# leakless21/VietVoice-TTS

Measured on AMD Instinct MI355X. Metric: audio-seconds/sec (24 kHz) at batch 32, 256-token utterances; RTF, higher is better.
Workload: dtype bf16

## Files before the change

### include/vvtts.h

```cpp
#ifndef VVTTS_H
#define VVTTS_H
#include <stddef.h>
#include <stdint.h>

#ifdef __cplusplus
extern "C" {
#endif

#if defined(__GNUC__)
#define VV_API __attribute__((visibility("default")))
#else
#define VV_API
#endif

#define VV_DTYPE_F32 0
#define VV_DTYPE_BF16 1
#define VV_MAX_UP 8
#define VV_MAX_RES 4

#define VV_ACT_NONE_ 0
#define VV_ACT_GELU_TANH_ 1
#define VV_ACT_GELU_ERF_ 2
#define VV_ACT_SILU_ 3
#define VV_ACT_MISH_ 4
// ... 103 lines not shown
    const float* t_host;
} vv_apg_args;
VV_API int vv_transformer_steps_apg(vv_ctx* ctx, const vv_steps_args* args, const uint8_t* guide_host, int ld_guide, const vv_apg_args* apg,
                                    void* stream);
VV_API int vv_transformer_apg_ws_bytes(vv_ctx* ctx, int B, int N, const int32_t* seq_len_host, uint64_t* bytes);

VV_API int vv_decode_ws_bytes(vv_ctx* ctx, int B, int t_gen_max, uint64_t* bytes);
VV_API int vv_decode_into(vv_ctx* ctx, int B, int N, const float* x, const int32_t* ref_signal_len, const int32_t* seq_len,
                   int t_gen_max, int16_t* pcm, int ld_pcm, int32_t* pcm_len, float* wave_f32, void* ws, uint64_t ws_bytes,
                   void* stream);
VV_API uint64_t vv_ws_generation(const vv_ctx* ctx);

VV_API int vv_set_rope_theta(vv_ctx* ctx, float theta);

VV_API int vv_set_option(vv_ctx* ctx, const char* name, int value);

#define VV_PROF_GEMM 0
#define VV_PROF_ATTN 1
#define VV_PROF_NORM 2
#define VV_PROF_POSCONV 3
#define VV_PROF_ELEMWISE 4
#define VV_PROF_VOC_CONV 5
#define VV_PROF_VOC_POST 6
#define VV_PROF_MEL 7
#define VV_PROF_TEXT 8
#define VV_PROF_VOC_PRE 9
#define VV_PROF_VOC_UP0 10
#define VV_PROF_VOC_MRF0 14
#define VV_PROF_NCLASS 18
VV_API int vv_prof_enable(vv_ctx* ctx, int on);
VV_API int vv_prof_collect(vv_ctx* ctx, int64_t* launches, double* ms, double* flops, double* bytes);

typedef struct vv_gemm_args {
    int32_t dtype, out_dtype, mode, act;
    const void* A; int32_t lda;
    const void* W; int32_t ldw;
    void* C; int32_t ldc;
    int32_t M, N, K;
    const float *bias, *gate, *cos_q, *sin_q, *cos_k, *sin_k;
    int32_t n_store, seq_n, rope_dim;
    const float *rope_cs_q, *rope_cs_k;
    int32_t tile;
    const int32_t* rope_pos;
    int32_t rope_by_row;
    int32_t tail_parts, tail_row0;
    void* C_tail;
    float rope_theta;
    int32_t rope_skip_q;
    int32_t chip_share;
} vv_gemm_args;
VV_API int vv_gemm(vv_ctx* ctx, const vv_gemm_args* args, void* stream);
VV_API int vv_gemm_tail_plan(vv_ctx* ctx, int32_t M, int32_t N, int32_t K, int32_t* row0, int32_t* parts);

typedef struct vv_attn_args {
    int32_t dtype;
    const void* qkv; int32_t ld_qkv;
    void* out; int32_t ld_out;
    int32_t n_seq, seq_n, heads, dim;
    const int32_t* kv_len;
    const int32_t* row_start;
    int32_t total_rows;
    float q_scale;
    const float* rope_cs_q;
} vv_attn_args;
VV_API int vv_attention(vv_ctx* ctx, const vv_attn_args* args, void* stream);

typedef struct vv_ln_args {
    int32_t out_dtype;
    const float* x; int32_t ldx;
    void* y; int32_t ldy;
    int32_t R, D;
    const float *w, *b;
    int32_t add_one;
    float eps;
    const void* delta;
    int32_t delta_dtype, ld_delta;
    const void* delta2;
    int32_t keep_x;
    int32_t tail_row0;
    int32_t delta_tail_parts, delta2_tail_parts;
    const void *delta_tail, *delta2_tail;
} vv_ln_args;
VV_API int vv_layernorm(vv_ctx* ctx, const vv_ln_args* args, void* stream);

typedef struct vv_posconv_args {
    int32_t dtype, out_dtype;
    const void* in; int32_t ld_in;
    const void* W;
    const float* bias;
    void* out; int32_t ld_out;
    const void* resid; int32_t ld_resid;
    int32_t n_seq, seq_n, groups, KW, B;
    const int32_t* seq_len;
    const int32_t* row_start;
} vv_posconv_args;
VV_API int vv_posconv(vv_ctx* ctx, const vv_posconv_args* args, void* stream);

typedef struct vv_conv_args {
    const float* in;
    const float* W;
    const float* bias;
    float* out;
    const float* resid;
    int32_t B, Cin, Cout, T_in, T_out, KW, dil, transposed, up, rows_total, rows_pad, accumulate;
    float pre_slope, out_scale;
    const int32_t* len_in;
    const void* W_x3;
    int32_t wg_rows;
} vv_conv_args;
VV_API int vv_conv1d(vv_ctx* ctx, const vv_conv_args* args, void* stream);
VV_API uint64_t vv_conv_split_bytes(int32_t Cin_pad, int32_t KW, int32_t rows_pad);
VV_API int vv_conv_split_weights(vv_ctx* ctx, const float* W, int32_t Cin_pad, int32_t KW, int32_t rows_pad, void* out, void* stream);

typedef struct vv_mrf_args {
    const float* y;
    const float *W1, *b1;
    const float *W2, *b2;
    float* out;
    int32_t B, C, T, KW, dil, rows_pad, accumulate;
    float slope, out_scale;
    const int32_t* len_in;
} vv_mrf_args;
VV_API int vv_mrf_resblock(vv_ctx* ctx, const vv_mrf_args* args, void* stream);

VV_API int vv_vocos_im2col(vv_ctx* ctx, const float* x, int B, int N, const int32_t* ref_signal_len, const int32_t* seq_len, int T_max,
                           float* out, int ld_out, void* stream);
VV_API int vv_istft_head(vv_ctx* ctx, int B, int T_max, const float* head, int ld_head, const int32_t* n_frames, int16_t* pcm, int ld_pcm,
                         int32_t* pcm_len, float* wave_f32, void* stream);
VV_API int vv_text_embed(vv_ctx* ctx, const int32_t* ids, int ld_ids, const int32_t* text_len, const float* emb, const float* pos,
                         int vocab_rows, float* out, int B, int N, int Dt, void* stream);
VV_API int vv_dwconv(vv_ctx* ctx, const float* in, float* out, const float* w, const float* bias, const int32_t* seq_len, int B, int n_seq,
                     int N, int C, int KW, void* stream);
VV_API int vv_grn(vv_ctx* ctx, int dtype, void* x, float* sumsq, const float* gamma, const float* beta, const int32_t* seq_len, int B,
                  int n_seq, int N, int C, void* stream);
VV_API int vv_conv_post(vv_ctx* ctx, const float* in, const float* w, float bias, int16_t* pcm, int ld_pcm, float* wave_f32,
                 int B, int C, int T, int KW, float pre_slope, const int32_t* len_in, void* stream);
VV_API int vv_mel(vv_ctx* ctx, const int16_t* audio, int ld_audio, const int32_t* audio_len, float* mel, int B, int F_max,
           void* stream);
VV_API int vv_groupnorm(vv_ctx* ctx, const float* x, float* y, const float* gamma, const float* beta, int B, int C, int T, int G,
                 float eps, int act, void* stream);
VV_API int vv_rope_compact(vv_ctx* ctx, const float* cos_t, const float* sin_t, float* out, int n, void* stream);
VV_API int vv_rope_rows(vv_ctx* ctx, const float* compact, const int32_t* pos, float* out, int rows, void* stream);
typedef struct vv_ode_stage_args {
    float* x; const float* pred; int32_t ldp, Rc, n_mel, n_prev;
    const float* k_prev[3]; float coef[4];
    float* k_out; float* x_out;
    float g; const float* g_item; int32_t seq_n; const int32_t* row_src;
} vv_ode_stage_args;
VV_API int vv_ode_stage(vv_ctx* ctx, const vv_ode_stage_args* args, void* stream);
VV_API int vv_ode_stage_guided(vv_ctx* ctx, const vv_ode_stage_args* args, const int32_t* u_row, void* stream);
typedef struct vv_apg_coef_args {
    const float* pred; int32_t ldp, Rc, n_mel;
    const int32_t* u_row;
    const float* x_e; const int32_t* row_src;
    int32_t B, n_tiles;
    const int32_t* row_start; const int32_t* len;
    float t_e, g;
    const float* g_item; const float* eta; const float* norm_rms;
    double* partials; float* coef;
} vv_apg_coef_args;
VV_API int vv_apg_coef(vv_ctx* ctx, const vv_apg_coef_args* args, void* stream);
typedef struct vv_apg_stage_args { const float* coef; const float* x_e; int32_t x_e_packed; float t_e; } vv_apg_stage_args;
VV_API int vv_ode_stage_apg(vv_ctx* ctx, const vv_ode_stage_args* args, const int32_t* u_row, const vv_apg_stage_args* apg, void* stream);
VV_API int vv_cfg_euler(vv_ctx* ctx, float* x, const float* pred, int ldp, int BN, int n_mel, float cfg, float dt, void* stream);

VV_API int vv_ingest_pcm(vv_ctx* ctx, const void* pcm, const int64_t* desc, int n_clips, int64_t max_out, float* out, void* stream);
// ... 56 lines not shown
```

### vietvoice-tts_amd/csrc/vv_api.hip

```cpp
#include <hip/hip_runtime.h>
#include <algorithm>
#include <cmath>
#include <cstdarg>
#include <cstdio>
#include <cstring>
#include <map>
#include <string>
#include <utility>
#include <vector>
#include "vv_kernels.h"

#define VV_VERSION_STR "vvtts-hip 0.9 (gfx950)"

namespace {
std::string g_create_error;

struct Bound { const void* p; uint64_t bytes; };

struct ProfRec { hipEvent_t a, b; int cls, sub; };

inline size_t align_up(size_t v, size_t a) { return (v + a - 1) / a * a; }
inline int pad_to(int v, int a) { return (v + a - 1) / a * a; }
}

struct vv_ctx {
    int device = 0;
    vv_model_cfg cfg{};
    int dt = VV_DTYPE_BF16;
    std::string err;
    std::map<std::string, Bound> w;
    bool finalized = false;
    bool ever_finalized = false;
    bool vocos = false;
    vv_vocos_cfg vcfg{};
    float post_bias = 0.f;
    int n_steps = 0;
    std::vector<float> dt_host;
    float* modtab = nullptr;
    float* fintab = nullptr;
    int ode_s = 1;
    double ode_a[16] = {}, ode_b[4] = {1.0, 0, 0, 0};
    int ode_kslot[4] = {-1, -1, -1, -1};
    int ode_nk = 0;
    char* ws = nullptr;
    size_t ws_cap = 0;
    uint64_t ws_generation = 0;
    int* d_mult = nullptr;
    int rope_rows = 0;
    int split_k_tail = 0;
    int chip_share = 1;
    int ring_tiles_max = 256;
    int ring_tiles = 1;
    int pp_min_tiles = -1;
    int lanes = 0;
    hipStream_t side_stream[1] = {};
    hipEvent_t ev_fork = nullptr, ev_join[1] = {};
    float rope_theta = 0.f;
    int rope_q_attn = 1;
    int voc_x3 = -1;
    int voc_x3_rows = 0;
    char* x3_buf = nullptr;
    std::map<std::string, const void*> x3_w;
    int fuse_mrf = 2;
    bool prof = false;
    std::vector<ProfRec> recs;
    std::vector<hipEvent_t> pool;
    int64_t p_launch[VV_PROF_NCLASS]{};
    double p_flops[VV_PROF_NCLASS]{}, p_bytes[VV_PROF_NCLASS]{}, p_ms[VV_PROF_NCLASS]{};

    int fail(int code, const char* fmt, ...) {
        char buf[1024];
        va_list ap;
        va_start(ap, fmt);
        vsnprintf(buf, sizeof buf, fmt, ap);
        va_end(ap);
        err = buf;
        return code;
    }
    const void* W(const std::string& n) const {
        auto it = w.find(n);
        return it == w.end() ? nullptr : it->second.p;
    }
    const float* Wf(const std::string& n) const { return (const float*)W(n); }
    int esz() const { return dt == VV_DTYPE_BF16 ? 2 : 4; }
    int bk() const { return dt == VV_DTYPE_BF16 ? 64 : 32; }
};

namespace {

#define HIPCHK(ctx, call)                                                                   \
    do {                                                                                    \
        hipError_t e__ = (call);                                                            \
        if (e__ != hipSuccess) return (ctx)->fail(-5, "%s: %s", #call, hipGetErrorString(e__)); \
    } while (0)

#define KCHK(ctx, call)                                              \
    do {                                                             \
        const char* m__ = "";                                        \
        int r__ = (call);                                            \
        if (r__ != 0) return (ctx)->fail(r__, "%s", m__);            \
    } while (0)

struct Prof {
    vv_ctx* c; int idx = -1; hipStream_t st;
    Prof(vv_ctx* c_, int cls, double flops, double bytes, hipStream_t st_, int sub = -1) : c(c_), st(st_) {
        if (!c->prof) return;
        ProfRec r; r.cls = cls; r.sub = sub;
        if (sub >= 0) { c->p_launch[sub]++; c->p_flops[sub] += flops; c->p_bytes[sub] += bytes; }
        auto get = [&]() { hipEvent_t e; if (!c->pool.empty()) { e = c->pool.back(); c->pool.pop_back(); } else hipEventCreate(&e); return e; };
        r.a = get(); r.b = get();
        hipEventRecord(r.a, st);
        c->recs.push_back(r); idx = (int)c->recs.size() - 1;
        c->p_launch[cls]++; c->p_flops[cls] += flops; c->p_bytes[cls] += bytes;
    }
    ~Prof() { if (idx >= 0) hipEventRecord(c->recs[idx].b, st); }
};

struct Arena {
    char* base = nullptr; size_t cap = 0, off = 0;
    template <typename T> T* take(size_t n) { off = align_up(off, 256); T* p = base ? (T*)(base + off) : nullptr; off += n * sizeof(T); return p; }
};
template <typename F> size_t plan_bytes(F&& plan) { Arena dry; plan(dry); return dry.off; }
int ensure_ws(vv_ctx* c, size_t bytes, Arena* a) {
    if (bytes > c->ws_cap) {
        if (c->ws) { hipDeviceSynchronize(); hipFree(c->ws); c->ws = nullptr; c->ws_cap = 0; }
        const size_t want = align_up(bytes + bytes / 16, 1 << 20);
        hipError_t e = hipMalloc((void**)&c->ws, want);
        if (e != hipSuccess) return c->fail(-12, "workspace hipMalloc(%zu MiB): %s", want >> 20, hipGetErrorString(e));
        c->ws_cap = want; ++c->ws_generation;
    }
    *a = Arena{c->ws, c->ws_cap, 0};
    return 0;
}
int use_ws(vv_ctx* c, void* block, size_t have, size_t need, Arena* a) {
    if ((uintptr_t)block % 256) return c->fail(-22, "workspace block must be 256-byte aligned");
    if (have < need) return c->fail(-22, "workspace block too small: %zu < %zu bytes", have, need);
    *a = Arena{(char*)block, have, 0};
    return 0;
}
template <typename F> int plan_ws(vv_ctx* c, void* block, size_t have, F&& plan) {
    const size_t need = plan_bytes(plan);
    Arena a;
    if (int r = block ? use_ws(c, block, have, need, &a) : ensure_ws(c, need, &a)) return r;
    plan(a);
    if (a.off > a.cap) return c->fail(-14, "workspace plan took %zu bytes of a %zu-byte block", a.off, a.cap);
    return 0;
}

struct Gemm : vv_gemm_args { const char* wname; };
Gemm gemm_args(const vv_ctx* c, int dtype, int out_dtype, int mode, int act, const void* A, int lda, const char* wname, int ldw,
               const char* bname, void* C, int ldc, int M, int N, int K) {
    Gemm g{};
    g.dtype = dtype; g.out_dtype = out_dtype; g.mode = mode; g.act = act;
    g.A = A; g.lda = lda; g.W = c->W(wname); g.ldw = ldw; g.C = C; g.ldc = ldc; g.M = M; g.N = N; g.K = K;
    g.bias = bname ? c->Wf(bname) : nullptr; g.wname = wname;
    if (bname && !g.bias) g.W = nullptr;
    return g;
}
int launch_gemm(vv_ctx* c, Gemm g, int cls, hipStream_t st, double alg_flops = -1) {
    if (!g.W) return c->fail(-2, "weight '%s' is not bound", g.wname);
    const int M = g.M, N = g.N, K = g.K, bf16 = g.dtype == VV_DTYPE_BF16;
    if (!g.chip_share) g.chip_share = c->chip_share;
    if (g.tile == 0 && c->pp_min_tiles >= 0 && bf16 && N % 256 == 0)
        g.tile = (M >= 4096 && (long long)((M + 255) / 256) * (N / 256) >= c->pp_min_tiles) ? 256 : 128;
    if (c->ring_tiles && g.tile == 0 && bf16 && N <= 1024 && N % 64 == 0 && (long long)((M + 63) / 64) * (N / 128) <= c->ring_tiles_max)
        g.tile = 6464;
    const int esz = bf16 ? 2 : 4, osz = g.out_dtype == VV_DTYPE_BF16 ? 2 : 4;
    const double fl = alg_flops >= 0 ? alg_flops : 2.0 * M * (double)N * K;
    Prof p(c, cls, fl, (double)M * K * esz + (double)N * K * esz + (double)M * N * osz * (g.mode == VV_EPI_GATE_RES ? 2 : 1), st);
    const char* m = "";
    if (int r = vvk_gemm(&g, st, &m)) return c->fail(r, "%s (weight %s, M=%d N=%d K=%d)", m, g.wname, M, N, K);
    return 0;
}

std::string blk(int i, const char* s) { return "blocks." + std::to_string(i) + s; }

}

extern "C" {

const char* vv_version(void) { return VV_VERSION_STR; }

const char* vv_last_error(const vv_ctx* ctx) { return ctx ? ctx->err.c_str() : g_create_error.c_str(); }

int vv_create(vv_ctx** out, int device, const vv_model_cfg* cfg, int acoustic_dtype) {
    if (!out || !cfg) { g_create_error = "vv_create: null argument"; return -22; }
    *out = nullptr;
    int n = 0;
    hipError_t e = hipGetDeviceCount(&n);
    if (e != hipSuccess || n <= 0) { g_create_error = "vv_create: no HIP device visible (the HIP path has no CPU fallback)"; return -19; }
    if (device < 0 || device >= n) { g_create_error = "vv_create: device index out of range"; return -22; }
    if (acoustic_dtype != VV_DTYPE_F32 && acoustic_dtype != VV_DTYPE_BF16) { g_create_error = "vv_create: dtype must be f32 or bf16"; return -22; }
    if (cfg->head_dim != 64 || cfg->heads * 64 != cfg->dim) { g_create_error = "vv_create: head_dim must be 64"; return -22; }
    if (cfg->dim % 128 || cfg->text_dim % 128 || cfg->dim / cfg->pos_conv_groups != 64 || cfg->n_mel % 4 || cfg->dim > 1024 ||
        cfg->text_dim > 1024) {
        g_create_error = "vv_create: dim/text_dim must be multiples of 128 (<=1024), 64 channels per pos-conv group"; return -22;
    }
    if (cfg->voc_n_up < 1 || cfg->voc_n_up > VV_MAX_UP || cfg->voc_n_res > VV_MAX_RES || cfg->voc_n_dil > VV_MAX_RES) {
        g_create_error = "vv_create: vocoder topology out of range"; return -22;
    }
    e = hipSetDevice(device);
    if (e != hipSuccess) { g_create_error = hipGetErrorString(e); return -5; }
    vv_ctx* c = new vv_ctx();
    c->device = device; c->cfg = *cfg; c->dt = acoustic_dtype;
    *out = c;
    return 0;
}

void vv_destroy(vv_ctx* c) {
    if (!c) return;
    hipSetDevice(c->device);
    hipDeviceSynchronize();
    if (c->ws) hipFree(c->ws);
    if (c->modtab) hipFree(c->modtab);
    if (c->fintab) hipFree(c->fintab);
    if (c->d_mult) hipFree(c->d_mult);
    if (c->x3_buf) hipFree(c->x3_buf);
    for (auto q : c->side_stream) if (q) hipStreamDestroy(q);
    if (c->ev_fork) hipEventDestroy(c->ev_fork);
    for (auto e : c->ev_join) if (e) hipEventDestroy(e);
    for (auto& r : c->recs) { hipEventDestroy(r.a); hipEventDestroy(r.b); }
    for (auto e : c->pool) hipEventDestroy(e);
    delete c;
}

int vv_bind_weight(vv_ctx* c, const char* name, const void* p, uint64_t bytes) {
    if (!c || !name || !p) return c ? c->fail(-22, "vv_bind_weight: null argument") : -22;
    if ((uintptr_t)p % 16) return c->fail(-22, "vv_bind_weight(%s): pointer must be 16-byte aligned", name);
    c->w[name] = Bound{p, bytes};
    c->finalized = false;
    return 0;
}

int vv_finalize_weights(vv_ctx* c) {
    if (!c) return -22;
    const vv_model_cfg& g = c->cfg;
    const int D = g.dim, Dt = g.text_dim, FF = g.dim * g.ff_mult, es = c->esz();
    const int KP = pad_to(2 * g.n_mel + Dt, 64), MP = pad_to(g.n_mel, 128);
    std::string missing;
    auto need = [&](const std::string& n, uint64_t bytes) {
        auto it = c->w.find(n);
        if (it == c->w.end()) { missing += n + " "; return; }
        if (it->second.bytes < bytes) missing += n + "(short:" + std::to_string(it->second.bytes) + "<" + std::to_string(bytes) + ") ";
    };
    need("const.window", 4ull * g.n_fft); need("const.tw_cos", 4ull * g.n_fft); need("const.tw_sin", 4ull * g.n_fft);
    need("const.mel_fb", 4ull * (g.n_fft / 2 + 1) * g.n_mel);
    need("const.text_pos", 4ull * g.max_pos * Dt);
    need("text.embed.weight", 4ull * g.vocab_rows * Dt);
    for (int i = 0; i < g.text_layers; ++i) {
        const std::string p = "text.blocks." + std::to_string(i);
        need(p + ".dwconv.weight", 4ull * Dt * g.text_conv_k); need(p + ".dwconv.bias", 4ull * Dt);
        need(p + ".norm.weight", 4ull * Dt); need(p + ".norm.bias", 4ull * Dt);
        need(p + ".pwconv1.weight", (uint64_t)es * Dt * g.text_ff_mult * Dt); need(p + ".pwconv1.bias", 4ull * Dt * g.text_ff_mult);
        need(p + ".grn.gamma", 4ull * Dt * g.text_ff_mult); need(p + ".grn.beta", 4ull * Dt * g.text_ff_mult);
        need(p + ".pwconv2.weight", (uint64_t)es * Dt * g.text_ff_mult * Dt); need(p + ".pwconv2.bias", 4ull * Dt);
    }
    need("input.proj.weight", (uint64_t)es * D * KP); need("input.proj.bias", 4ull * D);
    for (int j = 1; j <= 2; ++j) {
        need("input.pos_conv" + std::to_string(j) + ".weight", (uint64_t)es * D * 64 * g.pos_conv_k);
        need("input.pos_conv" + std::to_string(j) + ".bias", 4ull * D);
    }
    need("time.mlp1.weight", 4ull * D * g.time_freq_dim); need("time.mlp1.bias", 4ull * D);
    need("time.mlp2.weight", 4ull * D * D); need("time.mlp2.bias", 4ull * D);
    for (int i = 0; i < g.depth; ++i) {
        need(blk(i, ".adaln.weight"), 4ull * 6 * D * D); need(blk(i, ".adaln.bias"), 4ull * 6 * D);
        need(blk(i, ".attn.qkv.weight"), (uint64_t)es * 3 * D * D); need(blk(i, ".attn.qkv.bias"), 4ull * 3 * D);
        need(blk(i, ".attn.out.weight"), (uint64_t)es * D * D); need(blk(i, ".attn.out.bias"), 4ull * D);
        need(blk(i, ".ff1.weight"), (uint64_t)es * FF * D); need(blk(i, ".ff1.bias"), 4ull * FF);
        need(blk(i, ".ff2.weight"), (uint64_t)es * D * FF); need(blk(i, ".ff2.bias"), 4ull * D);
    }
    need("final.adaln.weight", 4ull * 2 * D * D); need("final.adaln.bias", 4ull * 2 * D);
    need("final.proj.weight", (uint64_t)es * MP * D); need("final.proj.bias", 4ull * MP);
    if (c->vocos) {
        const vv_vocos_cfg& v = c->vcfg;
        const uint64_t V = v.dim, I = v.intermediate, KE = pad_to(v.embed_k * g.n_mel, 32), HP = pad_to(v.n_fft + 2, 128);
        need("const.istft_basis", 4ull * v.n_fft * v.n_fft);
        need("voc.embed.weight", 4 * V * KE); need("voc.embed.bias", 4 * V);
        for (const char* n : {"voc.norm", "voc.final_norm"}) { need(std::string(n) + ".weight", 4 * V); need(std::string(n) + ".bias", 4 * V); }
        for (int i = 0; i < v.layers; ++i) {
            const std::string p = "voc.blocks." + std::to_string(i);
            need(p + ".dwconv.weight", 4 * V * v.dw_k); need(p + ".dwconv.bias", 4 * V);
            need(p + ".norm.weight", 4 * V); need(p + ".norm.bias", 4 * V);
            need(p + ".pwconv1.weight", 4 * I * V); need(p + ".pwconv1.bias", 4 * I);
            need(p + ".pwconv2.weight", 4 * V * I); need(p + ".pwconv2.bias", 4 * V);
            need(p + ".gamma", 4 * V);
        }
        need("voc.head.weight", 4 * HP * V); need("voc.head.bias", 4 * HP);
        if (!missing.empty()) return c->fail(-2, "missing or short weights: %s", missing.c_str());
        c->finalized = c->ever_finalized = true;
        return 0;
    }
    int ch = g.voc_pre_ch;
    struct ConvW { std::string name; int cin_pad, kw, rows_pad; };
    std::vector<ConvW> convs;
    convs.push_back({"voc.pre.weight", pad_to(g.n_mel, 8), g.voc_pre_k, pad_to(ch, 64)});
    need("voc.pre.weight", 4ull * pad_to(g.n_mel, 8) * g.voc_pre_k * pad_to(ch, 64)); need("voc.pre.bias", 4ull * ch);
    for (int s = 0; s < g.voc_n_up; ++s) {
        const int cin = ch, cout = ch / 2, u = g.voc_up_rates[s];
        const std::string p = "voc.up." + std::to_string(s);
        need(p + ".weight", 4ull * pad_to(cin, 8) * 2 * pad_to(cout * u, 64)); need(p + ".bias", 4ull * cout);
        convs.push_back({p + ".weight", pad_to(cin, 8), 2, pad_to(cout * u, 64)});
        for (int a = 0; a < g.voc_n_res; ++a)
            for (int b = 0; b < g.voc_n_dil; ++b)
// ... 637 lines not shown
        L.st = li == 0 ? st : c->side_stream[li - 1];
        L.row_start = L.tab; L.row_src = L.tab + 2 * L.B; L.row_pos = L.row_src + L.Rc;
        L.qkv_pos = L.uniform ? nullptr : L.row_pos;
    }
    const float rope_theta = c->dt == VV_DTYPE_BF16 ? c->rope_theta : 0.f;
    const int q_rope_attn = (c->rope_q_attn && c->dt == VV_DTYPE_BF16 && !(rope_theta > 0.f)) ? 1 : 0;

    auto setup = [&](Lane& L) -> int {
        hipStream_t st = L.st;
        KCHK(c, vvk_row_tables(L.seq_len, L.B, N, (int)L.Rc, L.tab, L.tab + 2 * L.B, L.tab + 2 * L.B + L.Rc, L.kv_len, st, &m__));
        KCHK(c, vvk_rope_compact(rope_cos_q, rope_sin_q, L.csq, N, st, &m__));
        KCHK(c, vvk_rope_compact(rope_cos_k, rope_sin_k, L.csk, N, st, &m__));
        if (guide) return 0;
        if (c->rope_rows) {
            KCHK(c, vvk_rope_rows(L.csq, L.row_pos, L.csq_rows, (int)L.R, st, &m__));
            KCHK(c, vvk_rope_rows(L.csk, L.row_pos, L.csk_rows, (int)L.R, st, &m__));
        }
        Prof p(c, VV_PROF_ELEMWISE, 0, 4.0 * L.R * (M + CD) / 2 + (double)es * L.R * KP, st);
        KCHK(c, vvk_pack_cat(c->dt, L.x, L.cat, L.cat_drop, L.xcat, KP, (int)L.Rc, M, CD, 0, L.row_src, st, &m__));
        return 0;
    };
    auto stage_state = [&](const Lane& L, int i) -> float* { return (apg && !(i & 1)) ? L.xs2 : L.xs; };
    auto step_pack = [&](Lane& L, int s, int i) -> int {
        hipStream_t st = L.st;
        const size_t Rc = L.Rc;
        if (s != step0 || i > 0) {
            Prof p(c, VV_PROF_ELEMWISE, 0, 4.0 * Rc * M + 2.0 * es * Rc * M, st);
            KCHK(c, vvk_pack_cat(c->dt, i ? stage_state(L, i) : L.x, L.cat, L.cat_drop, L.xcat, KP, (int)Rc, M, CD, 1, i ? nullptr : L.row_src, st, &m__));
        }
        return 0;
    };
    auto guide_eval = [&](Lane& L, GuideState& G, int i, int e) -> int {
        hipStream_t st = L.st;
        const uint8_t* row = guide + (size_t)e * ld_guide + L.b0;
        std::vector<uint8_t> f(L.B);
        size_t Ru = 0; int Bu = 0; double sq = 0;
        for (int b = 0; b < L.B; ++b) {
            f[b] = row[b] ? 1 : 0;
            if (f[b]) { Ru += hlen[L.b0 + b]; ++Bu; sq += (double)hlen[L.b0 + b] * hlen[L.b0 + b]; }
        }
        const bool first = G.flags.empty(), changed = first || f != G.flags;
        if (changed) {
            KCHK(c, vvk_guided_tables(L.seq_len, f.data(), L.B, N, (int)L.Rc, (int)Ru, L.g_row_start, L.g_rs_rel, L.g_kv_len, L.g_row_pos, L.u_src,
                                      L.u_crow, L.u_row, st, &m__));
            if (c->rope_rows) {
                KCHK(c, vvk_rope_rows(L.csq, L.g_row_pos, L.csq_rows, (int)(L.Rc + Ru), st, &m__));
                KCHK(c, vvk_rope_rows(L.csk, L.g_row_pos, L.csk_rows, (int)(L.Rc + Ru), st, &m__));
            }
            G.flags = f; G.Ru = Ru; G.Bu = Bu; G.sum_sq = sq;
        }
        const float* xin = i ? stage_state(L, i) : L.x;
        const int Rc = (int)L.Rc, R = (int)(L.Rc + Ru);
        auto pack = [&](int row0, int n_rows, int only_x) -> int {
            Prof p(c, VV_PROF_ELEMWISE, 0, only_x ? (4.0 + es) * n_rows * M : 4.0 * n_rows * (M + CD) + (double)es * n_rows * KP, st);
            KCHK(c, vvk_pack_cat_guided(c->dt, xin, L.cat, L.cat_drop, L.xcat, KP, Rc, row0, n_rows, M, CD, only_x, i ? 1 : 0, L.row_src, L.u_src,
                                        L.u_crow, st, &m__));
            return 0;
        };
        if (first || !changed) return pack(0, R, first ? 0 : 1);
        if (int r = pack(0, Rc, 1)) return r;
        return Ru ? pack(Rc, (int)Ru, 0) : 0;
    };
    auto step_head = [&](Lane& L, int s) -> int {
        (void)s;
        hipStream_t st = L.st;
        const size_t R = L.R;
        Gemm proj = gemm_args(c, c->dt, c->dt, VV_EPI_STORE, VV_ACT_NONE_, L.xcat, KP, "input.proj.weight", KP, "input.proj.bias", L.h, D, (int)R, D, KP);
        if (int r = launch_gemm(c, proj, VV_PROF_GEMM, st, 2.0 * R * D * (M + CD))) return r;
        for (int j = 1; j <= 2; ++j) {
            vv_posconv_args a{};
            a.dtype = c->dt; a.out_dtype = (j == 1) ? c->dt : VV_DTYPE_F32;
            a.in = (j == 1) ? L.h : L.h2; a.ld_in = D;
            const std::string wn = "input.pos_conv" + std::to_string(j) + ".weight", bn = "input.pos_conv" + std::to_string(j) + ".bias";
            a.W = c->W(wn); a.bias = c->Wf(bn);
            a.out = (j == 1) ? (void*)L.h2 : (void*)L.xres; a.ld_out = D;
            a.resid = (j == 2) ? L.h : nullptr; a.ld_resid = D;
            a.n_seq = L.n_seq; a.seq_n = N; a.groups = g.pos_conv_groups; a.KW = g.pos_conv_k; a.B = L.n_seq; a.seq_len = L.kv_len; a.row_start = L.row_start;
            Prof p(c, VV_PROF_POSCONV, 2.0 * R * D * 64 * g.pos_conv_k, (double)es * R * D * 2 + (j == 2 ? 4.0 * R * D : 0), st);
            KCHK(c, vvk_posconv(&a, st, &m__));
        }
        L.pending = false;
        return 0;
    };
    auto block = [&](Lane& L, int s, int l) -> int {
        hipStream_t st = L.st;
        const size_t R = L.R;
        const bool pending = L.pending;
        const float* mod = c->modtab + ((size_t)l * S + s) * 6 * D;
        const std::string qkvw = blk(l, ".attn.qkv.weight"), qkvb = blk(l, ".attn.qkv.bias"), ow = blk(l, ".attn.out.weight"),
                          ob = blk(l, ".attn.out.bias"), f1w = blk(l, ".ff1.weight"), f1b = blk(l, ".ff1.bias"),
                          f2w = blk(l, ".ff2.weight"), f2b = blk(l, ".ff2.bias");
        vv_ln_args a{}; a.out_dtype = c->dt; a.x = L.xres; a.ldx = D; a.y = L.h; a.ldy = D; a.R = (int)R; a.D = D; a.add_one = 1; a.eps = 1e-6f;
        a.delta_dtype = c->dt; a.ld_delta = D;
        a.tail_row0 = L.tail_row0; a.delta_tail = L.h2_tail; a.delta2_tail = L.h3_tail;
        a.delta_tail_parts = pending ? L.tp_o : 0; a.delta2_tail_parts = pending ? L.tp_f : 0;
        a.w = mod + D; a.b = mod;
        a.delta = pending ? L.h2 : nullptr; a.delta2 = pending ? L.h3 : nullptr; a.keep_x = 0;
        { Prof p(c, VV_PROF_NORM, 0, (4.0 + es) * R * D + (pending ? (4.0 + 2.0 * es) * R * D : 0), st); KCHK(c, vvk_ln_mod(&a, st, &m__)); }
        Gemm qkv = gemm_args(c, c->dt, c->dt, VV_EPI_QKV_ROPE, VV_ACT_NONE_, L.h, D, qkvw.c_str(), D, qkvb.c_str(), L.qkv, 3 * D, (int)R, 3 * D, D);
        qkv.cos_q = rope_cos_q; qkv.sin_q = rope_sin_q; qkv.cos_k = rope_cos_k; qkv.sin_k = rope_sin_k;
        qkv.rope_cs_q = c->rope_rows ? L.csq_rows : L.csq; qkv.rope_cs_k = c->rope_rows ? L.csk_rows : L.csk; qkv.rope_by_row = c->rope_rows;
        qkv.seq_n = N; qkv.rope_dim = D; qkv.rope_pos = L.qkv_pos; qkv.rope_skip_q = q_rope_attn; qkv.rope_theta = rope_theta;
        if (int r = launch_gemm(c, qkv, VV_PROF_GEMM, st)) return r;
        {
            vv_attn_args t{}; t.dtype = c->dt; t.qkv = L.qkv; t.ld_qkv = 3 * D; t.out = L.att; t.ld_out = D; t.n_seq = L.n_seq; t.seq_n = N;
            t.heads = g.heads; t.dim = D; t.kv_len = L.kv_len; t.row_start = L.row_start; t.total_rows = (int)R;
            t.rope_cs_q = q_rope_attn ? L.csq : nullptr;
            t.q_scale = rope_theta > 0.f ? 1.0f / sqrtf((float)g.head_dim) : 0.f;
            Prof p(c, VV_PROF_ATTN, 4.0 * g.heads * L.sum_sq * 64, (double)es * R * 4 * D, st);
            KCHK(c, vvk_attention(&t, st, &m__));
        }
        Gemm out = gemm_args(c, c->dt, c->dt, VV_EPI_GATE_STORE, VV_ACT_NONE_, L.att, D, ow.c_str(), D, ob.c_str(), L.h2, D, (int)R, D, D);
        out.gate = mod + 2 * D;
        if (L.tp_o) { out.C_tail = L.h2_tail; out.tail_row0 = L.tail_row0; out.tail_parts = L.tp_o; }
        if (int r = launch_gemm(c, out, VV_PROF_GEMM, st)) return r;
        a.w = mod + 4 * D; a.b = mod + 3 * D;
        a.delta = L.h2; a.delta2 = nullptr; a.keep_x = 1; a.delta_tail_parts = L.tp_o; a.delta2_tail_parts = 0;
        { Prof p(c, VV_PROF_NORM, 0, (4.0 + 2.0 * es) * R * D, st); KCHK(c, vvk_ln_mod(&a, st, &m__)); }
        if (int r = launch_gemm(c, gemm_args(c, c->dt, c->dt, VV_EPI_STORE, VV_ACT_GELU_TANH_, L.h, D, f1w.c_str(), D, f1b.c_str(), L.ffm, FF, (int)R, FF, D), VV_PROF_GEMM, st)) return r;
        Gemm ff2 = gemm_args(c, c->dt, c->dt, VV_EPI_GATE_STORE, VV_ACT_NONE_, L.ffm, FF, f2w.c_str(), FF, f2b.c_str(), L.h3, D, (int)R, D, FF);
        ff2.gate = mod + 5 * D;
        if (L.tp_f) { ff2.C_tail = L.h3_tail; ff2.tail_row0 = L.tail_row0; ff2.tail_parts = L.tp_f; }
        if (int r = launch_gemm(c, ff2, VV_PROF_GEMM, st)) return r;
        L.pending = true;
        return 0;
    };
    auto step_tail = [&](Lane& L, int s) -> int {
        hipStream_t st = L.st;
        const size_t R = L.R;
        const bool pending = L.pending;
        {
            const float* fm = c->fintab + (size_t)s * 2 * D;
            vv_ln_args a{}; a.out_dtype = c->dt; a.x = L.xres; a.ldx = D; a.y = L.h; a.ldy = D; a.R = (int)R; a.D = D; a.add_one = 1; a.eps = 1e-6f;
            a.w = fm; a.b = fm + D;
            a.delta = pending ? L.h2 : nullptr; a.delta2 = pending ? L.h3 : nullptr; a.keep_x = 1;
            a.delta_dtype = c->dt; a.ld_delta = D;
            a.tail_row0 = L.tail_row0; a.delta_tail = L.h2_tail; a.delta2_tail = L.h3_tail;
            a.delta_tail_parts = pending ? L.tp_o : 0; a.delta2_tail_parts = pending ? L.tp_f : 0;
            Prof p(c, VV_PROF_NORM, 0, es * R * D + (pending ? (4.0 + 2.0 * es) * R * D : 4.0 * R * D), st);
            KCHK(c, vvk_ln_mod(&a, st, &m__));
        }
        Gemm proj = gemm_args(c, c->dt, VV_DTYPE_F32, VV_EPI_STORE, VV_ACT_NONE_, L.h, D, "final.proj.weight", D, "final.proj.bias", L.pred, MP, (int)R, MP, D);
        proj.n_store = M;
        return launch_gemm(c, proj, VV_PROF_GEMM, st, 2.0 * R * D * M);
    };
    auto step_euler = [&](Lane& L, int s) -> int {
        hipStream_t st = L.st;
        Prof p(c, VV_PROF_ELEMWISE, 0, 16.0 * L.Rc * M, st);
        KCHK(c, vvk_cfg_euler(L.x, L.pred, MP, (int)L.Rc, M, g.cfg_strength, c->dt_host[s], L.row_src, st, &m__));
        return 0;
    };
    auto step_stage = [&](Lane& L, int s, int i) -> int {
        hipStream_t st = L.st;
        const bool last = i == ns - 1;
        const double h = (double)c->dt_host[s];
        vv_ode_stage_args a{};
        a.x = L.x; a.pred = L.pred; a.ldp = MP; a.Rc = (int)L.Rc; a.n_mel = M; a.n_prev = i;
        int n_read = 0;
        for (int j = 0; j <= i; ++j) {
            a.coef[j] = (float)(h * (last ? c->ode_b[j] : c->ode_a[(i + 1) * 4 + j]));
            if (j < i && a.coef[j] != 0.f) { a.k_prev[j] = L.kbuf[c->ode_kslot[j]]; ++n_read; }
        }
        a.k_out = (!last && c->ode_kslot[i] >= 0) ? L.kbuf[c->ode_kslot[i]] : nullptr;
        a.x_out = last ? nullptr : stage_state(L, i + 1);
        a.g = g.cfg_strength; a.g_item = cfg_item ? cfg_item + L.b0 : nullptr; a.seq_n = N; a.row_src = L.row_src;
        const int* u_row = guide ? L.u_row : nullptr;
        vv_apg_stage_args sa{};
        if (apg) {
            vv_apg_coef_args q{};
            q.pred = L.pred; q.ldp = MP; q.Rc = (int)L.Rc; q.n_mel = M; q.u_row = u_row;
            q.x_e = i ? stage_state(L, i) : L.x; q.row_src = i ? nullptr : L.row_src;
            q.B = L.B; q.n_tiles = (N + VV_APG_TILE - 1) / VV_APG_TILE; q.row_start = L.row_start; q.len = L.kv_len;
            q.t_e = apg->t_host[s * ns + i]; q.g = a.g; q.g_item = a.g_item;
            q.eta = apg->eta ? apg->eta + L.b0 : nullptr; q.norm_rms = apg->norm_rms ? apg->norm_rms + L.b0 : nullptr;
            q.partials = L.apg_part; q.coef = L.apg_coef;
            { Prof p(c, VV_PROF_ELEMWISE, 14.0 * L.Rc * M, 12.0 * L.Rc * M, st); KCHK(c, vvk_apg_coef(&q, 1, st, &m__)); }
            { Prof p(c, VV_PROF_ELEMWISE, 0, 24.0 * L.B * q.n_tiles, st); KCHK(c, vvk_apg_coef(&q, 2, st, &m__)); }
            sa.coef = L.apg_coef; sa.x_e = q.x_e; sa.x_e_packed = i ? 1 : 0; sa.t_e = q.t_e;
        }
        Prof p(c, VV_PROF_ELEMWISE, 0, 4.0 * L.Rc * M * (4 + n_read + (a.k_out ? 1 : 0) + (apg ? 1 : 0)), st);
        KCHK(c, vvk_ode_stage(&a, u_row, apg ? &sa : nullptr, st, &m__));
        return 0;
    };

    Lane views[2];
    int n_views = n_lanes;
    auto branch_view = [&](const Lane& L, int v) {
        Lane V = L;
        const size_t r0 = v ? L.Rc : 0;
        V.st = v ? c->side_stream[0] : st;
        V.R = L.Rc; V.n_seq = L.B; V.sum_sq = L.sum_sq / 2;
        V.xcat += r0 * KP * es; V.h += r0 * D * es; V.h2 += r0 * D * es; V.h3 += r0 * D * es; V.att += r0 * D * es;
        V.qkv += r0 * 3 * D * es; V.ffm += r0 * FF * es; V.xres += r0 * D; V.pred += r0 * MP;
        V.csq_rows += r0 * 64; V.csk_rows += r0 * 64;
        return V;
    };
    if (branch_lanes) {
        n_views = 2;
        for (int v = 0; v < 2; ++v) views[v] = branch_view(lanes[0], v);
    } else {
        for (int li = 0; li < n_lanes; ++li) views[li] = lanes[li];
    }
    GuideState gstate[2];
    auto guided_views = [&]() {
        if (branch_lanes) {
            const Lane& L = lanes[0];
            const GuideState& G = gstate[0];
            n_views = G.Ru ? 2 : 1;
            for (int v = 0; v < n_views; ++v) {
                Lane& V = views[v];
                V = branch_view(L, v);
                V.row_start = v ? L.g_rs_rel : L.g_row_start; V.kv_len = v ? L.g_kv_len + L.B : L.g_kv_len;
                V.qkv_pos = L.uniform ? nullptr : (v ? L.g_row_pos + L.Rc : L.g_row_pos);
                if (v) { V.R = G.Ru; V.n_seq = G.Bu; V.sum_sq = G.sum_sq; }
            }
            return;
        }
        for (int li = 0; li < n_lanes; ++li) {
            Lane& V = views[li];
            const GuideState& G = gstate[li];
            V = lanes[li];
            V.R = V.Rc + G.Ru; V.n_seq = V.B + G.Bu; V.sum_sq = V.sum_sq / 2 + G.sum_sq;
            V.row_start = V.g_row_start; V.kv_len = V.g_kv_len; V.qkv_pos = V.uniform ? nullptr : V.g_row_pos;
        }
    };
    auto fork = [&]() -> int {
        HIPCHK(c, hipEventRecord(c->ev_fork, st));
        HIPCHK(c, hipStreamWaitEvent(c->side_stream[0], c->ev_fork, 0));
        return 0;
    };
    auto join = [&]() {
        hipEventRecord(c->ev_join[0], c->side_stream[0]);
        hipStreamWaitEvent(st, c->ev_join[0], 0);
    };
    int rc = 0;
    c->chip_share = n_views;
    if (n_lanes > 1) rc = fork();
    for (int li = 0; li < n_lanes && !rc; ++li) rc = setup(lanes[li]);
    for (int s = step0; s < step0 + n_steps && !rc; ++s)
        for (int i = 0; i < ns && !rc; ++i) {
            const int e = s * ns + i;
            if (guide) {
                for (int li = 0; li < n_lanes && !rc; ++li) rc = guide_eval(lanes[li], gstate[li], i, e);
                guided_views();
                c->chip_share = n_views;
            } else {
                for (int li = 0; li < n_lanes && !rc; ++li) rc = step_pack(lanes[li], s, i);
            }
            const bool want_fork = branch_lanes && n_views == 2;
            if (want_fork && !rc) rc = fork();
            const bool forked = want_fork && !rc;
            for (int v = 0; v < n_views && !rc; ++v) rc = step_head(views[v], e);
            for (int l = 0; l < g.depth && !rc; ++l)
                for (int v = 0; v < n_views && !rc; ++v) rc = block(views[v], e, l);
            for (int v = 0; v < n_views && !rc; ++v) rc = step_tail(views[v], e);
            if (forked) join();
            for (int li = 0; li < n_lanes && !rc; ++li) rc = rk ? step_stage(lanes[li], s, i) : step_euler(lanes[li], s);
        }
    if (n_lanes > 1) join();
    c->chip_share = 1;
    return rc;
}

static vv_steps_args steps_args(int B, int N, const int32_t* seq_len, const int32_t* seq_len_host, float* x, const float* cat, const float* cat_drop,
                                const float* rope_cos_q, const float* rope_sin_q, const float* rope_cos_k, const float* rope_sin_k, int step0, int n_steps) {
    vv_steps_args a{};
    a.B = B; a.N = N; a.seq_len = seq_len; a.seq_len_host = seq_len_host; a.x = x; a.cat_mel_text = cat; a.cat_mel_text_drop = cat_drop;
    a.rope_cos_q = rope_cos_q; a.rope_sin_q = rope_sin_q; a.rope_cos_k = rope_cos_k; a.rope_sin_k = rope_sin_k; a.step0 = step0; a.n_steps = n_steps;
    return a;
}

int vv_transformer_steps(vv_ctx* c, int B, int N, const int32_t* seq_len, float* x, const float* cat, const float* cat_drop,
                         const float* rope_cos_q, const float* rope_sin_q, const float* rope_cos_k, const float* rope_sin_k,
                         int step0, int n_steps, void* stream) {
    return transformer_steps_impl(c, steps_args(B, N, seq_len, nullptr, x, cat, cat_drop, rope_cos_q, rope_sin_q, rope_cos_k, rope_sin_k, step0, n_steps), nullptr, stream);
}

int vv_transformer_steps_h(vv_ctx* c, int B, int N, const int32_t* seq_len, const int32_t* seq_len_host, float* x, const float* cat,
                           const float* cat_drop, const float* rope_cos_q, const float* rope_sin_q, const float* rope_cos_k,
                           const float* rope_sin_k, int step0, int n_steps, void* stream) {
    if (c && !seq_len_host) return c->fail(-22, "vv_transformer_steps_h: host lengths missing");
    return transformer_steps_impl(c, steps_args(B, N, seq_len, seq_len_host, x, cat, cat_drop, rope_cos_q, rope_sin_q, rope_cos_k, rope_sin_k, step0, n_steps), nullptr, stream);
}

int vv_transformer_ws_bytes(vv_ctx* c, int B, int N, const int32_t* seq_len_host, uint64_t* bytes) {
    if (c && (!seq_len_host || !bytes)) return c->fail(-22, "vv_transformer_ws_bytes: bad arguments");
    vv_steps_args a{};
    a.B = B; a.N = N; a.seq_len_host = seq_len_host;
    return transformer_steps_impl(c, a, bytes, nullptr);
}

int vv_transformer_steps_into(vv_ctx* c, int B, int N, const int32_t* seq_len, const int32_t* seq_len_host, float* x, const float* cat,
                              const float* cat_drop, const float* rope_cos_q, const float* rope_sin_q, const float* rope_cos_k,
                              const float* rope_sin_k, int step0, int n_steps, void* ws, uint64_t ws_bytes, void* stream) {
    if (c && (!seq_len_host || !ws)) return c->fail(-22, "vv_transformer_steps_into: host lengths and a workspace block are required");
    vv_steps_args a = steps_args(B, N, seq_len, seq_len_host, x, cat, cat_drop, rope_cos_q, rope_sin_q, rope_cos_k, rope_sin_k, step0, n_steps);
    a.ws = ws; a.ws_bytes = ws_bytes;
    return transformer_steps_impl(c, a, nullptr, stream);
}

int vv_transformer_steps_ex(vv_ctx* c, const vv_steps_args* a, void* stream) {
    if (!c) return -22;
    if (!a) return c->fail(-22, "vv_transformer_steps_ex: null arguments");
    if (a->ws && !a->seq_len_host) return c->fail(-22, "vv_transformer_steps_ex: a workspace block needs the host lengths");
    if (a->cfg_item && (uintptr_t)a->cfg_item % 4) return c->fail(-22, "vv_transformer_steps_ex: cfg_item must be a float array");
    return transformer_steps_impl(c, *a, nullptr, stream);
}

int vv_transformer_steps_guided(vv_ctx* c, const vv_steps_args* a, const uint8_t* guide_host, int ld_guide, void* stream) {
    if (!guide_host) return vv_transformer_steps_ex(c, a, stream);
    if (!c) return -22;
    if (!a) return c->fail(-22, "vv_transformer_steps_guided: null arguments");
    if (a->ws && !a->seq_len_host) return c->fail(-22, "vv_transformer_steps_guided: a workspace block needs the host lengths");
    if (a->cfg_item && (uintptr_t)a->cfg_item % 4) return c->fail(-22, "vv_transformer_steps_guided: cfg_item must be a float array");
    return transformer_steps_impl(c, *a, nullptr, stream, guide_host, ld_guide, false);
}

int vv_transformer_guided_ws_bytes(vv_ctx* c, int B, int N, const int32_t* seq_len_host, uint64_t* bytes) {
    if (c && (!seq_len_host || !bytes)) return c->fail(-22, "vv_transformer_guided_ws_bytes: bad arguments");
    vv_steps_args a{};
    a.B = B; a.N = N; a.seq_len_host = seq_len_host;
    return transformer_steps_impl(c, a, bytes, nullptr, nullptr, 0, true);
}

int vv_transformer_steps_apg(vv_ctx* c, const vv_steps_args* a, const uint8_t* guide_host, int ld_guide, const vv_apg_args* apg, void* stream) {
    if (!apg) return vv_transformer_steps_guided(c, a, guide_host, ld_guide, stream);
    if (!c) return -22;
    if (!a) return c->fail(-22, "vv_transformer_steps_apg: null arguments");
    if (a->ws && !a->seq_len_host) return c->fail(-22, "vv_transformer_steps_apg: a workspace block needs the host lengths");
    if (a->cfg_item && (uintptr_t)a->cfg_item % 4) return c->fail(-22, "vv_transformer_steps_apg: cfg_item must be a float array");
    if (!apg->t_host) return c->fail(-22, "vv_transformer_steps_apg: the evaluation times t_host are required");
    if (((uintptr_t)apg->eta | (uintptr_t)apg->norm_rms) % 4) return c->fail(-22, "vv_transformer_steps_apg: eta and norm_rms must be float arrays");
    return transformer_steps_impl(c, *a, nullptr, stream, guide_host, ld_guide, false, apg, false);
}

int vv_transformer_apg_ws_bytes(vv_ctx* c, int B, int N, const int32_t* seq_len_host, uint64_t* bytes) {
    if (c && (!seq_len_host || !bytes)) return c->fail(-22, "vv_transformer_apg_ws_bytes: bad arguments");
    vv_steps_args a{};
// ... 146 lines not shown
        const char* m = "";
        int r = vvk_conv(&a, st, &m);
        if (r) return c->fail(r, "%s (%s)", m, name.c_str());
        return 0;
    };
    if (int r = conv(v0, "voc.pre", buf[0], nullptr, M, Cs[0], Ts[0], Ts[0], g.voc_pre_k, 1, 0, 1.0f, 1.0f, 0, lens, VV_PROF_VOC_PRE)) return r;
    float* cur = buf[0];
    float* up_out = buf[1];
    for (int s = 0; s < nu; ++s) {
        const int C = Cs[s + 1], T = Ts[s + 1];
        const int* len_s = lens + (size_t)(s + 1) * B;
        if (int r = conv(cur, "voc.up." + std::to_string(s), up_out, nullptr, Cs[s], C, Ts[s], T, 2, 1, g.voc_up_rates[s], g.voc_lrelu, 1.0f, 0, lens + (size_t)s * B,
                         s < 4 ? VV_PROF_VOC_UP0 + s : -1)) return r;
        float* acc = cur;
        float* t1 = (up_out == buf[1]) ? buf[2] : buf[1];
        float* ya = buf[3];
        float* yb = buf[4];
        const float inv = 1.0f / (float)g.voc_n_res;
        const int mrf_cls = s < 4 ? VV_PROF_VOC_MRF0 + s : -1;
        for (int a = 0; a < g.voc_n_res; ++a) {
            const float* y = up_out;
            for (int b = 0; b < g.voc_n_dil; ++b) {
                const std::string q = "voc.res." + std::to_string(s) + "." + std::to_string(a) + "." + std::to_string(b);
                const bool last = b == g.voc_n_dil - 1;
                float* dst = last ? acc : ((y == ya) ? yb : ya);
                const int kw = g.voc_res_kernels[a], dil = g.voc_res_dilations[b];
                if ((c->fuse_mrf == 1 || (c->fuse_mrf == 2 && B <= 8 && !x3)) && (C == 32 || C == 64) && (kw == 3 || kw == 7 || kw == 11)) {
                    vv_mrf_args m{};
                    m.y = y; m.W1 = c->Wf(q + ".conv1.weight"); m.b1 = c->Wf(q + ".conv1.bias"); m.W2 = c->Wf(q + ".conv2.weight"); m.b2 = c->Wf(q + ".conv2.bias");
                    m.out = dst; m.B = B; m.C = C; m.T = T; m.KW = kw; m.dil = dil; m.rows_pad = 64; m.accumulate = last && a > 0;
                    m.slope = g.voc_lrelu; m.out_scale = last ? inv : 1.0f; m.len_in = len_s;
                    Prof p(c, VV_PROF_VOC_CONV, 2.0 * 2.0 * B * (double)T * C * C * kw, 4.0 * B * (double)C * T * (2 + (m.accumulate ? 1 : 0)), st, mrf_cls);
                    const char* em = "";
                    if (int r = vvk_mrf_pair(&m, st, &em)) return c->fail(r, "%s (%s)", em, q.c_str());
                } else {
                    if (int r = conv(y, q + ".conv1", t1, nullptr, C, C, T, T, kw, dil, 0, g.voc_lrelu, 1.0f, 0, len_s, mrf_cls)) return r;
                    if (int r = conv(t1, q + ".conv2", dst, y, C, C, T, T, kw, 1, 0, g.voc_lrelu, last ? inv : 1.0f, last && a > 0, len_s, mrf_cls)) return r;
                }
                y = dst;
            }
        }
    }
    {
        const int C = Cs[nu], T = Ts[nu];
        Prof p(c, VV_PROF_VOC_POST, 2.0 * B * (double)T * C * g.voc_post_k, 4.0 * B * (double)C * T + 2.0 * B * T, st);
        KCHK(c, vvk_conv_post(cur, c->Wf("voc.post.weight"), c->post_bias, pcm, ld_pcm, wave_f32, B, C, T, g.voc_post_k, 0.01f,
                              lens + (size_t)nu * B, st, &m__));
    }
    return 0;
}

int vv_set_rope_theta(vv_ctx* c, float theta) {
    if (!c) return -22;
    if (theta != 0.f && !(theta > 1.f)) return c->fail(-22, "vv_set_rope_theta: the base must be > 1 (0 = read the tables)");
    c->rope_theta = theta;
    return 0;
}

int vv_set_option(vv_ctx* c, const char* name, int value) {
    if (!c || !name) return -22;
    if (!strcmp(name, "rope_rows")) { c->rope_rows = value != 0; return 0; }
    if (!strcmp(name, "rope_q_attn")) { c->rope_q_attn = value != 0; return 0; }
    if (!strcmp(name, "voc_x3_rows")) {
        if (value != 0 && value != 128) return c->fail(-22, "vv_set_option: voc_x3_rows takes 0 (64-row workgroups) or 128");
        c->voc_x3_rows = value; return 0;
    }
    if (!strcmp(name, "voc_x3")) {
        if (value < -1 || value > 1) return c->fail(-22, "vv_set_option: voc_x3 takes -1 (by acoustic dtype), 0 (f32 MFMA) or 1 (3-way bf16 split)");
        c->voc_x3 = value; return 0;
    }
    if (!strcmp(name, "split_k_tail")) {
        if (value < 0 || value > 2) return c->fail(-22, "vv_set_option: split_k_tail takes 0 (off), 1 (out-projection and FF2) or 2 (FF2 only)");
        c->split_k_tail = value; return 0;
    }
    if (!strcmp(name, "ring_tiles")) { c->ring_tiles = value != 0; if (value > 1) c->ring_tiles_max = value; return 0; }
    if (!strcmp(name, "pp_min_tiles")) {
        if (value < -1) return c->fail(-22, "vv_set_option: pp_min_tiles takes -1 (the launcher's rule) or a 256-tile count >= 0");
        c->pp_min_tiles = value; return 0;
    }
    if (!strcmp(name, "lanes")) {
        if (value < 0 || value > 2) return c->fail(-22, "vv_set_option: lanes takes 0 (auto), 1 (one lane) or 2 (two lanes whenever the batch has two items)");
        c->lanes = value; return 0;
    }
    if (!strcmp(name, "fuse_mrf")) {
        if (value < 0 || value > 2) return c->fail(-22, "vv_set_option: fuse_mrf takes 0 (off), 1 (on) or 2 (auto)");
        c->fuse_mrf = value; return 0;
    }
    return c->fail(-22, "vv_set_option: unknown option '%s'", name);
}

int vv_decode(vv_ctx* c, int B, int N, const float* x, const int32_t* ref_len, const int32_t* seq_len, int t_gen_max, int16_t* pcm,
              int ld_pcm, int32_t* pcm_len, float* wave_f32, void* stream) {
    return decode_impl(c, B, N, x, ref_len, seq_len, t_gen_max, pcm, ld_pcm, pcm_len, wave_f32, nullptr, 0, stream);
}

int vv_decode_into(vv_ctx* c, int B, int N, const float* x, const int32_t* ref_len, const int32_t* seq_len, int t_gen_max, int16_t* pcm,
                   int ld_pcm, int32_t* pcm_len, float* wave_f32, void* ws, uint64_t ws_bytes, void* stream) {
    if (!c) return -22;
    if (!ws) return c->fail(-22, "vv_decode_into: null workspace block");
    return decode_impl(c, B, N, x, ref_len, seq_len, t_gen_max, pcm, ld_pcm, pcm_len, wave_f32, ws, ws_bytes, stream);
}

int vv_prof_enable(vv_ctx* c, int on) {
    if (!c) return -22;
    c->prof = on != 0;
    return 0;
}
int vv_prof_collect(vv_ctx* c, int64_t* launches, double* ms, double* flops, double* bytes) {
    if (!c) return -22;
    hipSetDevice(c->device);
    HIPCHK(c, hipDeviceSynchronize());
    for (auto& r : c->recs) {
        float t = 0.f;
        if (hipEventElapsedTime(&t, r.a, r.b) == hipSuccess) { c->p_ms[r.cls] += t; if (r.sub >= 0) c->p_ms[r.sub] += t; }
        c->pool.push_back(r.a); c->pool.push_back(r.b);
    }
    c->recs.clear();
    for (int i = 0; i < VV_PROF_NCLASS; ++i) {
        if (launches) launches[i] = c->p_launch[i];
        if (ms) ms[i] = c->p_ms[i];
        if (flops) flops[i] = c->p_flops[i];
        if (bytes) bytes[i] = c->p_bytes[i];
        c->p_launch[i] = 0; c->p_ms[i] = 0; c->p_flops[i] = 0; c->p_bytes[i] = 0;
    }
    return 0;
}

#define SINGLE(ctx, call)                                     \
    do {                                                      \
        if (!(ctx)) return -22;                               \
        hipSetDevice((ctx)->device);                          \
        const char* m__ = "";                                 \
        int r__ = (call);                                     \
        if (r__) return (ctx)->fail(r__, "%s", m__);          \
        return 0;                                             \
    } while (0)

int vv_gemm(vv_ctx* c, const vv_gemm_args* a, void* st) { SINGLE(c, vvk_gemm(a, (hipStream_t)st, &m__)); }
int vv_gemm_tail_plan(vv_ctx* c, int32_t M, int32_t N, int32_t K, int32_t* row0, int32_t* parts) {
    if (!row0 || !parts || M < 1 || N < 1 || K < 1) return c ? c->fail(-22, "vv_gemm_tail_plan: bad arguments") : -22;
    if (c) HIPCHK(c, hipSetDevice(c->device));
    vvk_gemm_tail_plan(M, N, K, K, K, N, row0, parts);
    return 0;
}
int vv_attention(vv_ctx* c, const vv_attn_args* a, void* st) { SINGLE(c, vvk_attention(a, (hipStream_t)st, &m__)); }
int vv_layernorm(vv_ctx* c, const vv_ln_args* a, void* st) { SINGLE(c, vvk_ln_mod(a, (hipStream_t)st, &m__)); }
int vv_posconv(vv_ctx* c, const vv_posconv_args* a, void* st) { SINGLE(c, vvk_posconv(a, (hipStream_t)st, &m__)); }
int vv_conv1d(vv_ctx* c, const vv_conv_args* a, void* st) { SINGLE(c, vvk_conv(a, (hipStream_t)st, &m__)); }
uint64_t vv_conv_split_bytes(int32_t Cin_pad, int32_t KW, int32_t rows_pad) {
    return (Cin_pad < 1 || KW < 1 || rows_pad < 1) ? 0 : (uint64_t)vvk_conv_split_bytes(Cin_pad, KW, rows_pad);
}
int vv_conv_split_weights(vv_ctx* c, const float* W, int32_t Cin_pad, int32_t KW, int32_t rows_pad, void* out, void* st) {
    SINGLE(c, vvk_conv_split_weights(W, Cin_pad, KW, rows_pad, out, (hipStream_t)st, &m__));
}
int vv_mrf_resblock(vv_ctx* c, const vv_mrf_args* a, void* st) { SINGLE(c, vvk_mrf_pair(a, (hipStream_t)st, &m__)); }
int vv_conv_post(vv_ctx* c, const float* in, const float* w, float bias, int16_t* pcm, int ld_pcm, float* wave_f32, int B, int C, int T,
                 int KW, float pre_slope, const int32_t* len_in, void* st) {
    SINGLE(c, vvk_conv_post(in, w, bias, pcm, ld_pcm, wave_f32, B, C, T, KW, pre_slope, len_in, (hipStream_t)st, &m__));
}
int vv_mel(vv_ctx* c, const int16_t* audio, int ld_audio, const int32_t* audio_len, float* mel, int B, int F_max, void* st) {
    if (!c) return -22;
    if (!c->W("const.window") || !c->W("const.tw_cos") || !c->W("const.tw_sin") || !c->W("const.mel_fb"))
        return c->fail(-2, "vv_mel: constant tables not bound");
    SINGLE(c, vvk_mel(audio, ld_audio, audio_len, c->Wf("const.window"), c->Wf("const.tw_cos"), c->Wf("const.tw_sin"), c->Wf("const.mel_fb"),
                      mel, B, F_max, c->cfg.n_fft, c->cfg.hop_length, c->cfg.n_mel, (hipStream_t)st, &m__));
}
int vv_groupnorm(vv_ctx* c, const float* x, float* y, const float* gamma, const float* beta, int B, int C, int T, int G, float eps, int act, void* st) {
    SINGLE(c, vvk_groupnorm(x, y, gamma, beta, B, C, T, G, eps, act, (hipStream_t)st, &m__));
}
int vv_rope_rows(vv_ctx* c, const float* compact, const int32_t* pos, float* out, int rows, void* st) {
    SINGLE(c, vvk_rope_rows(compact, pos, out, rows, (hipStream_t)st, &m__));
}
int vv_rope_compact(vv_ctx* c, const float* cos_t, const float* sin_t, float* out, int n, void* st) {
    SINGLE(c, vvk_rope_compact(cos_t, sin_t, out, n, (hipStream_t)st, &m__));
}
int vv_resample_poly(vv_ctx* c, const float* x, int n_in, const double* taps, int n_taps, int up, int down, int skip, float* y, int n_out, void* st) {
    SINGLE(c, vvk_resample_poly(x, n_in, taps, n_taps, up, down, skip, y, n_out, (hipStream_t)st, &m__));
}
int vv_ingest_pcm(vv_ctx* c, const void* pcm, const int64_t* desc, int n_clips, int64_t max_out, float* out, void* st) {
    SINGLE(c, vvk_ingest_pcm(pcm, (const long long*)desc, n_clips, (long long)max_out, out, (hipStream_t)st, &m__));
}
size_t vv_normalize_scratch_bytes(int n_clips, int64_t total_len) { return vvk_normalize_scratch_bytes(n_clips, (long long)total_len); }
int vv_normalize_clips(vv_ctx* c, const float* x, const int64_t* offsets, int n_clips, int64_t max_len, void* scratch, int16_t* out, void* st) {
    SINGLE(c, vvk_normalize_clips(x, (const long long*)offsets, n_clips, (long long)max_len, scratch, out, (hipStream_t)st, &m__));
}
int vv_vocos_im2col(vv_ctx* c, const float* x, int B, int N, const int32_t* ref_len, const int32_t* seq_len, int T_max, float* out, int ld_out,
                    void* st) {
    if (c && !c->vocos) return c->fail(-22, "vv_vocos_im2col: not a Vocos context (vv_set_vocos)");
    SINGLE(c, vvk_vocos_im2col(x, B, N, c->cfg.n_mel, ref_len, seq_len, T_max, c->vcfg.embed_k, out, ld_out, (hipStream_t)st, &m__));
}
int vv_istft_head(vv_ctx* c, int B, int T_max, const float* head, int ld_head, const int32_t* n_frames, int16_t* pcm, int ld_pcm, int32_t* pcm_len,
                  float* wave_f32, void* stream) {
    if (!c) return -22;
    if (!c->vocos || !c->finalized) return c->fail(-22, "vv_istft_head: needs a finalized Vocos context");
    if (B < 1 || T_max < 1 || !head || !n_frames || !pcm || ld_head < c->vcfg.n_fft + 2 || ld_pcm < T_max * c->vcfg.hop_length)
        return c->fail(-22, "vv_istft_head: bad arguments (ld_head >= n_fft + 2, ld_pcm >= T_max * hop)");
    if ((size_t)B * T_max * c->vcfg.n_fft * 4 >= ((size_t)1 << 31)) return c->fail(-22, "vv_istft_head: a plane of 2 GiB or more");
    hipSetDevice(c->device);
    const size_t R = (size_t)B * T_max;
    float *spec, *frames;
    if (int r = plan_ws(c, nullptr, 0, [&](Arena& a) { spec = a.take<float>(R * c->vcfg.n_fft); frames = a.take<float>(R * c->vcfg.n_fft); })) return r;
    return vocos_istft(c, B, T_max, head, ld_head, n_frames, pcm, ld_pcm, pcm_len, wave_f32, spec, frames, (hipStream_t)stream);
}
int vv_ode_stage(vv_ctx* c, const vv_ode_stage_args* a, void* st) {
    if (!c || !a) return c ? c->fail(-22, "vv_ode_stage: null arguments") : -22;
    SINGLE(c, vvk_ode_stage(a, nullptr, nullptr, (hipStream_t)st, &m__));
}
int vv_ode_stage_guided(vv_ctx* c, const vv_ode_stage_args* a, const int32_t* u_row, void* st) {
    if (!c || !a) return c ? c->fail(-22, "vv_ode_stage_guided: null arguments") : -22;
    if ((uintptr_t)u_row % 4) return c->fail(-22, "vv_ode_stage_guided: u_row must be an int32 array");
    SINGLE(c, vvk_ode_stage(a, u_row, nullptr, (hipStream_t)st, &m__));
}
int vv_ode_stage_apg(vv_ctx* c, const vv_ode_stage_args* a, const int32_t* u_row, const vv_apg_stage_args* apg, void* st) {
    if (!apg) return vv_ode_stage_guided(c, a, u_row, st);
    if (!c || !a) return c ? c->fail(-22, "vv_ode_stage_apg: null arguments") : -22;
    if ((uintptr_t)u_row % 4) return c->fail(-22, "vv_ode_stage_apg: u_row must be an int32 array");
    SINGLE(c, vvk_ode_stage(a, u_row, apg, (hipStream_t)st, &m__));
}
int vv_apg_coef(vv_ctx* c, const vv_apg_coef_args* a, void* st) {
    if (!c || !a) return c ? c->fail(-22, "vv_apg_coef: null arguments") : -22;
    if (((uintptr_t)a->u_row | (uintptr_t)a->row_src | (uintptr_t)a->row_start | (uintptr_t)a->len | (uintptr_t)a->g_item | (uintptr_t)a->eta |
         (uintptr_t)a->norm_rms) % 4)
        return c->fail(-22, "vv_apg_coef: the index and item arrays must be 4-byte aligned");
    SINGLE(c, vvk_apg_coef(a, 3, (hipStream_t)st, &m__));
}
int vv_text_embed(vv_ctx* c, const int32_t* ids, int ld_ids, const int32_t* text_len, const float* emb, const float* pos, int vocab_rows,
                  float* out, int B, int N, int Dt, void* st) {
    if (!c) return -22;
    if (!ids || !text_len || !emb || !pos || !out || B < 1 || N < 1 || ld_ids < 1 || vocab_rows < 1 || Dt < 4 || Dt % 4)
// ... 30 lines not shown
```

### vietvoice-tts_amd/csrc/vv_attention.hip

```cpp
#include "vv_common.h"
#include "vv_kernels.h"

namespace {

constexpr float LOG2E = 1.4426950408889634f;
constexpr float NEG_BIG = -1.0e30f;
constexpr float RESCALE_SUM = 1.8446744073709552e19f;
constexpr float TINY_SUM = 5.421010862427522e-20f;

__device__ __forceinline__ float fast_exp2(float x) { return __builtin_amdgcn_exp2f(x); }
__device__ __forceinline__ float half_max(float v) {
    const auto r = __builtin_amdgcn_permlane32_swap(__float_as_uint(v), __float_as_uint(v), false, false);
    float d;
    asm("v_max_f32 %0, %1, %2" : "=v"(d) : "v"(__uint_as_float(r[0])), "v"(__uint_as_float(r[1])));
    return d;
}
__device__ __forceinline__ float bf16_round(float v) {
    const unsigned u = __float_as_uint(v);
    return __uint_as_float((u + 0x7FFFu + ((u >> 16) & 1u)) & 0xFFFF0000u);
}
__device__ __forceinline__ bf16x8 make_q_ext(float v, int h) {
    bf16x8 f;
#pragma unroll
    for (int j = 0; j < 8; ++j) f[j] = (bf16)0.f;
    f[0] = (bf16)(h == 0 ? v : 0.f);
    return f;
}
__device__ __forceinline__ float half_sum(float v) {
    const auto r = __builtin_amdgcn_permlane32_swap(__float_as_uint(v), __float_as_uint(v), false, false);
    return __uint_as_float(r[0]) + __uint_as_float(r[1]);
}

typedef __attribute__((ext_vector_type(4))) int i32x4_t;
__device__ __forceinline__ i32x4_t make_rsrc4(const void* base, unsigned bytes) {
    const unsigned long long a = (unsigned long long)base;
    i32x4_t r;
    r[0] = __builtin_amdgcn_readfirstlane((int)(unsigned)a);
    r[1] = __builtin_amdgcn_readfirstlane((int)(unsigned)((a >> 32) & 0xffffu));
    r[2] = __builtin_amdgcn_readfirstlane((int)bytes);
    r[3] = 0x00020000;
    return r;
}
__device__ __forceinline__ void glds16_buf_asm(i32x4_t rs, unsigned voff, unsigned lds_dst) {
    unsigned keep;
    asm volatile("s_mov_b32 %0, m0\n\ts_mov_b32 m0, %3\n\ts_nop 0\n\tbuffer_load_dwordx4 %1, %2, 0 offen lds\n\ts_mov_b32 m0, %0"
                 : "=&s"(keep) : "v"(voff), "s"(rs), "s"(lds_dst) : "memory");
}

struct AttnBlock { int qb, head, seq; bool valid; };
__device__ __forceinline__ AttnBlock attn_block(int nqb, int heads, int n_seq) {
    const int b = blockIdx.x;
    const int xcd = b & 7, j = b >> 3;
    const int pair = (j / nqb) * 8 + xcd;
    AttnBlock r;
    r.qb = j % nqb;
    r.valid = pair < heads * n_seq;
    r.head = pair % heads;
    r.seq = pair / heads;
    return r;
}

#ifndef VV_ATTN_ABLATE
#define VV_ATTN_ABLATE 0
#endif

__global__ __launch_bounds__(256, 2) void attn_bf16_kernel(const bf16* __restrict__ qkv, int ld, bf16* __restrict__ out,
                                                           int ldo, int seq_n, int D, const int* __restrict__ kv_len_arr,
                                                           const int* __restrict__ row_start, int total_rows, int heads, int n_seq,
                                                           const float* __restrict__ rope_cs_q, float q_mul) {
    __shared__ __attribute__((aligned(16))) char smem[2 * 16384];
    const AttnBlock blk = attn_block((seq_n + 127) / 128, heads, n_seq);
    if (!blk.valid) return;
    const int head = blk.head, seq = blk.seq, qblock = blk.qb;
    const int lane = threadIdx.x & 63;
    const int wave = __builtin_amdgcn_readfirstlane(threadIdx.x >> 6);
    const int r32 = lane & 31, h = lane >> 5;
    int kv_len = kv_len_arr ? kv_len_arr[seq] : seq_n;
    if (row_start && kv_len <= 0) return;
    kv_len = max(1, min(kv_len, seq_n));
    const size_t row0 = row_start ? (size_t)row_start[seq] : (size_t)seq * seq_n;
    const int q_lim = row_start ? kv_len : seq_n;
    if (qblock * 128 >= q_lim) return;

    const bf16* Qp = qkv + row0 * ld + head * 64;
    const bf16* Kp = Qp + D;
    const unsigned kv_bytes = (unsigned)(((size_t)total_rows - row0) * (size_t)ld * 2 - (size_t)(head * 64 + D) * 2);

    const int q0 = qblock * 128 + wave * 32;
    const int qrow = min(q0 + r32, q_lim - 1);
    bf16x8 qf[4];
#pragma unroll
    for (int ds = 0; ds < 4; ++ds) {
        qf[ds] = *(const bf16x8*)(Qp + (size_t)qrow * ld + ds * 16 + h * 8);
        if (rope_cs_q) {
            const float* tq = rope_cs_q + (size_t)qrow * 64 + ds * 16 + h * 8;
            const float4 t0 = *(const float4*)tq, t1 = *(const float4*)(tq + 4);
            const float cs[8] = {t0.x, t0.y, t0.z, t0.w, t1.x, t1.y, t1.z, t1.w};
#pragma unroll
            for (int j = 0; j < 8; j += 2) {
                const float a = (float)qf[ds][j], b = (float)qf[ds][j + 1];
                const float na = __builtin_fmaf(a, cs[j], -(b * cs[j + 1])), nb = __builtin_fmaf(b, cs[j], a * cs[j + 1]);
                qf[ds][j] = (bf16)(na * LOG2E);
                qf[ds][j + 1] = (bf16)(nb * LOG2E);
            }
        } else {
#pragma unroll
            for (int j = 0; j < 8; ++j) qf[ds][j] = (bf16)((float)qf[ds][j] * q_mul);
        }
    }

    const i32x4_t rs4 = make_rsrc4(Kp, kv_bytes);
    const unsigned lds0 = (unsigned)(size_t)(lptr_t)smem;
    unsigned voff_k[2], voff_v[2];
#pragma unroll
    for (int u = 0; u < 2; ++u) {
        const int row = (wave * 2 + u) * 8 + (lane >> 3);
        const int p = lane & 7;
        const int ck = p ^ ((row >> 1) & 7);
        const int cv = p ^ (((row >> 1) & 1) << 2);
        voff_k[u] = (unsigned)row * (unsigned)ld * 2u + ck * 16;
        voff_v[u] = (unsigned)row * (unsigned)ld * 2u + (unsigned)D * 2u + cv * 16;
    }
    const int tile_bytes = 64 * ld * 2;
    auto stage = [&](int kt, int buf) {
#pragma unroll
        for (int u = 0; u < 2; ++u) {
            const int q = wave * 2 + u;
            glds16_buf_asm(rs4, voff_k[u] + kt * tile_bytes, lds0 + buf * 16384 + q * 1024);
            glds16_buf_asm(rs4, voff_v[u] + kt * tile_bytes, lds0 + buf * 16384 + 8192 + q * 1024);
        }
    };

    f32x16 o[2];
#pragma unroll
    for (int i = 0; i < 2; ++i)
#pragma unroll
        for (int r = 0; r < 16; ++r) o[i][r] = 0.f;
    float m_eff = 0.f, l_run = 0.f;
    bool has_ref = false;
    f32x16 zero16;
#pragma unroll
    for (int r = 0; r < 16; ++r) zero16[r] = 0.f;
    const bf16x8 k_one = make_q_ext(1.0f, h);
    bf16x8 q_ext = make_q_ext(0.f, h);

    const int tr_grp = (lane >> 4) & 1, tr_i = lane & 15, tr_q = tr_i >> 2, tr_p = tr_i & 3;
    int tr_off[2];
#pragma unroll
    for (int dt = 0; dt < 2; ++dt) {
        const int c = dt * 4 + 2 * tr_grp + (tr_p >> 1);
        tr_off[dt] = (4 * h + tr_q) * 128 + ((c ^ (((tr_q >> 1) & 1) << 2)) << 4) + (tr_p & 1) * 8;
    }

    const int n_tiles = (kv_len + 63) / 64;
    stage(0, 0);
    for (int kt = 0; kt < n_tiles; ++kt) {
        asm volatile("s_waitcnt vmcnt(0)" ::: "memory");
        __syncthreads();
// ... 63 lines not shown
        scores();
        psum = exps();
        if (kt + 1 < n_tiles) stage(kt + 1, (kt + 1) & 1);
        redo = __any(!(psum <= RESCALE_SUM));
        if (kt == 0) redo = redo || __any(!(half_sum(psum) >= TINY_SUM));
        if (redo) {
            scores();
            float mx = s[0][0];
#pragma unroll
            for (int kb = 0; kb < 2; ++kb)
#pragma unroll
                for (int r = 0; r < 16; ++r) mx = fmaxf(mx, s[kb][r]);
            mx = half_max(mx);
            const float m_new = bf16_round(m_eff + (kt == 0 ? mx : fmaxf(mx, 0.f)));
            const float d = m_new - m_eff;
            if (kt != 0) {
                const float alpha = fast_exp2(-d);
                l_run *= alpha;
#pragma unroll
                for (int dt = 0; dt < 2; ++dt)
#pragma unroll
                    for (int r = 0; r < 16; ++r) o[dt][r] *= alpha;
            }
#pragma unroll
            for (int kb = 0; kb < 2; ++kb)
#pragma unroll
                for (int r = 0; r < 16; ++r) s[kb][r] -= d;
            m_eff = m_new;
            q_ext = make_q_ext(-m_new, h);
            has_ref = true;
            psum = exps();
        }
#endif
        l_run += psum;
#if VV_ATTN_ABLATE == 3
        continue;
#endif

        __builtin_amdgcn_s_setprio(1);
#pragma unroll
        for (int kb = 0; kb < 2; ++kb)
#pragma unroll
            for (int st = 0; st < 2; ++st) {
                const f32x8 pv = {s[kb][8 * st + 0], s[kb][8 * st + 1], s[kb][8 * st + 2], s[kb][8 * st + 3],
                                  s[kb][8 * st + 4], s[kb][8 * st + 5], s[kb][8 * st + 6], s[kb][8 * st + 7]};
#if VV_ATTN_ABLATE == 1
                typedef __attribute__((ext_vector_type(4))) float f32x4a;
                const bf16x8 pf = __builtin_bit_cast(bf16x8, (f32x4a){pv[0], pv[2], pv[4], pv[6]});
#else
                const bf16x8 pf = __builtin_convertvector(pv, bf16x8);
#endif
#if VV_ATTN_ABLATE == 2
                asm volatile("" :: "v"(pf));
                continue;
#endif
#pragma unroll
                for (int dt = 0; dt < 2; ++dt) {
                    const char* a0 = sV + tr_off[dt] + (kb * 32 + 16 * st) * 128;
                    const char* a1 = a0 + 8 * 128;
                    const bf16x4 v0 = __builtin_amdgcn_ds_read_tr16_b64_v4bf16((__attribute__((address_space(3))) bf16x4*)a0);
                    const bf16x4 v1 = __builtin_amdgcn_ds_read_tr16_b64_v4bf16((__attribute__((address_space(3))) bf16x4*)a1);
                    const bf16x8 vf = {v0[0], v0[1], v0[2], v0[3], v1[0], v1[1], v1[2], v1[3]};
                    o[dt] = __builtin_amdgcn_mfma_f32_32x32x16_bf16(vf, pf, o[dt], 0, 0, 0);
                }
            }
        __builtin_amdgcn_s_setprio(0);
    }
    const float l_tot = half_sum(l_run);
    const float inv = 1.0f / l_tot;
    const int q = q0 + r32;
    if (q < q_lim) {
        bf16* op = out + (row0 + q) * ldo + head * 64;
#pragma unroll
        for (int dt = 0; dt < 2; ++dt)
#pragma unroll
            for (int g = 0; g < 4; ++g) {
                const int d0 = dt * 32 + 8 * g + 4 * h;
                store4<bf16>(op + d0, o[dt][4 * g] * inv, o[dt][4 * g + 1] * inv, o[dt][4 * g + 2] * inv,
                             o[dt][4 * g + 3] * inv);
            }
    }
}

__global__ __launch_bounds__(256, 2) void attn_f32_kernel(const float* __restrict__ qkv, int ld, float* __restrict__ out,
                                                          int ldo, int seq_n, int D, const int* __restrict__ kv_len_arr,
                                                          const int* __restrict__ row_start, int heads, int n_seq) {
    __shared__ __attribute__((aligned(16))) char smem[2 * 32768];
    const AttnBlock blk = attn_block((seq_n + 127) / 128, heads, n_seq);
    if (!blk.valid) return;
    const int head = blk.head, seq = blk.seq, qblock = blk.qb;
    const int lane = threadIdx.x & 63;
    const int wave = __builtin_amdgcn_readfirstlane(threadIdx.x >> 6);
    const int r32 = lane & 31, h = lane >> 5;
    int kv_len = kv_len_arr ? kv_len_arr[seq] : seq_n;
    if (row_start && kv_len <= 0) return;
    kv_len = max(1, min(kv_len, seq_n));
    const size_t row0 = row_start ? (size_t)row_start[seq] : (size_t)seq * seq_n;
    const int q_lim = row_start ? kv_len : seq_n;
    if (qblock * 128 >= q_lim) return;

    const float* Qp = qkv + row0 * ld + head * 64;
    const float* Kp = Qp + D;
    const float* Vp = Qp + 2 * D;

    const int q0 = qblock * 128 + wave * 32;
    const int qrow = min(q0 + r32, q_lim - 1);
    f32x4 qf[8];
#pragma unroll
    for (int kk = 0; kk < 8; ++kk) qf[kk] = *(const f32x4*)(Qp + (size_t)qrow * ld + kk * 8 + h * 4);

    auto stage = [&](int kt, int buf) {
        char* base = smem + buf * 32768;
#pragma unroll
        for (int u = 0; u < 4; ++u) {
            const int q = wave * 4 + u;
            const int row = q * 4 + (lane >> 4);
            const int key = min(kt * 64 + row, q_lim - 1);
            const int p = lane & 15;
            const int ck = p ^ (row & 15);
            glds16(Kp + (size_t)key * ld + ck * 4, base + q * 1024);
            glds16(Vp + (size_t)key * ld + p * 4, base + 16384 + q * 1024);
        }
    };

    f32x16 o[2];
#pragma unroll
    for (int i = 0; i < 2; ++i)
#pragma unroll
        for (int r = 0; r < 16; ++r) o[i][r] = 0.f;
    float m_run = NEG_BIG, l_run = 0.f;

    const int n_tiles = (kv_len + 63) / 64;
    stage(0, 0);
    for (int kt = 0; kt < n_tiles; ++kt) {
        asm volatile("s_waitcnt vmcnt(0)" ::: "memory");
        __syncthreads();
        if (kt + 1 < n_tiles) stage(kt + 1, (kt + 1) & 1);
        const char* sK = smem + (kt & 1) * 32768;
        const char* sV = sK + 16384;

        f32x16 s[2];
#pragma unroll
        for (int kb = 0; kb < 2; ++kb) {
#pragma unroll
            for (int r = 0; r < 16; ++r) s[kb][r] = 0.f;
            const int row = kb * 32 + r32;
#pragma unroll
            for (int kk = 0; kk < 8; ++kk) {
                const f32x4 kf = *(const f32x4*)(sK + row * 256 + (((2 * kk + h) ^ (row & 15)) << 4));
#pragma unroll
                for (int j = 0; j < 4; ++j)
                    s[kb] = __builtin_amdgcn_mfma_f32_32x32x2f32(kf[j], qf[kk][j], s[kb], 0, 0, 0);
            }
        }
        const int kbase = kt * 64;
        if (kbase + 64 > kv_len) {
#pragma unroll
            for (int kb = 0; kb < 2; ++kb)
#pragma unroll
                for (int r = 0; r < 16; ++r) {
                    const int key = kbase + kb * 32 + (r & 3) + 8 * (r >> 2) + 4 * h;
                    if (key >= kv_len) s[kb][r] = NEG_BIG;
                }
        }
        float mx = s[0][0];
#pragma unroll
        for (int kb = 0; kb < 2; ++kb)
#pragma unroll
            for (int r = 0; r < 16; ++r) mx = fmaxf(mx, s[kb][r]);
        mx = fmaxf(mx, __shfl_xor(mx, 32));
        const float m_new = fmaxf(m_run, mx);
        const float alpha = exp2f((m_run - m_new) * LOG2E);
        m_run = m_new;
        const float msc = m_new * LOG2E;
        float psum = 0.f;
#pragma unroll
        for (int kb = 0; kb < 2; ++kb)
#pragma unroll
            for (int r = 0; r < 16; ++r) {
                const float p = exp2f(fmaf(s[kb][r], LOG2E, -msc));
                psum += p;
                s[kb][r] = p;
            }
        l_run = l_run * alpha + psum;
#pragma unroll
        for (int dt = 0; dt < 2; ++dt)
#pragma unroll
            for (int r = 0; r < 16; ++r) o[dt][r] *= alpha;

#pragma unroll
        for (int kb = 0; kb < 2; ++kb)
#pragma unroll
            for (int i = 0; i < 16; ++i) {
                const int key = kb * 32 + (i & 3) + 8 * (i >> 2) + 4 * h;
#pragma unroll
                for (int dt = 0; dt < 2; ++dt) {
                    const float vf = *(const float*)(sV + key * 256 + (dt * 32 + r32) * 4);
                    o[dt] = __builtin_amdgcn_mfma_f32_32x32x2f32(vf, s[kb][i], o[dt], 0, 0, 0);
                }
            }
    }
    const float l_tot = l_run + __shfl_xor(l_run, 32);
    const float inv = 1.0f / l_tot;
    const int q = q0 + r32;
    if (q < q_lim) {
        float* op = out + (row0 + q) * ldo + head * 64;
#pragma unroll
        for (int dt = 0; dt < 2; ++dt)
#pragma unroll
            for (int g = 0; g < 4; ++g) {
                const int d0 = dt * 32 + 8 * g + 4 * h;
                store4<float>(op + d0, o[dt][4 * g] * inv, o[dt][4 * g + 1] * inv, o[dt][4 * g + 2] * inv,
                              o[dt][4 * g + 3] * inv);
            }
    }
}

}

int vvk_attention(const vv_attn_args* a, hipStream_t st, const char** err) {
    if (a->n_seq <= 0 || a->seq_n <= 0 || a->heads <= 0) { *err = "attention: empty shape"; return -22; }
    if (a->dim != a->heads * 64) { *err = "attention: head_dim must be 64"; return -22; }
    const int esz = a->dtype == VV_BF16 ? 2 : 4;
    if (((size_t)a->ld_qkv * esz) % 16 || ((size_t)a->ld_out * esz) % (4 * esz) || ((uintptr_t)a->qkv % 16) || ((uintptr_t)a->out % 16)) {
        *err = "attention: qkv/out must be 16-byte aligned (ld_out: 4 elements)"; return -22;
    }
    if (a->ld_qkv < 3 * a->dim || a->ld_out < a->dim) { *err = "attention: leading dimensions too small"; return -22; }
    if (a->row_start && !a->kv_len) { *err = "attention: packed rows need kv_len"; return -22; }
    if (a->rope_cs_q && (a->dtype != VV_BF16 || ((uintptr_t)a->rope_cs_q % 16))) { *err = "attention: the query-side rope table is taken by the bf16 kernel only, 16-byte aligned"; return -22; }
    if (a->row_start && a->total_rows <= 0) { *err = "attention: packed rows need total_rows (rows in the qkv buffer)"; return -22; }
    const int total_rows = a->total_rows > 0 ? a->total_rows : a->n_seq * a->seq_n;
    if (a->dtype == VV_BF16 && (size_t)total_rows * a->ld_qkv * 2 >= ((size_t)1 << 31)) { *err = "attention: qkv buffer must stay below 2 GiB"; return -22; }
    if (a->row_start == nullptr && total_rows < a->n_seq * a->seq_n) { *err = "attention: total_rows smaller than n_seq * seq_n"; return -22; }
    const int nqb = (a->seq_n + 127) / 128;
    const long long pairs8 = ((long long)a->heads * a->n_seq + 7) / 8;
    if (pairs8 * nqb * 8 > 0x7fffffffLL) { *err = "attention: grid too large"; return -22; }
    const dim3 grid((unsigned)(pairs8 * nqb * 8));
    if (a->dtype == VV_BF16)
        attn_bf16_kernel<<<grid, 256, 0, st>>>((const bf16*)a->qkv, a->ld_qkv, (bf16*)a->out, a->ld_out, a->seq_n, a->dim, a->kv_len, a->row_start, total_rows,
                                               a->heads, a->n_seq, a->rope_cs_q, LOG2E * (a->q_scale > 0.f ? a->q_scale : 1.0f));
    else
        attn_f32_kernel<<<grid, 256, 0, st>>>((const float*)a->qkv, a->ld_qkv, (float*)a->out, a->ld_out, a->seq_n, a->dim, a->kv_len, a->row_start,
                                              a->heads, a->n_seq);
    hipError_t he = hipGetLastError();
    if (he != hipSuccess) { *err = hipGetErrorString(he); return -5; }
    return 0;
}
```

### vietvoice-tts_amd/csrc/vv_elementwise.hip

```cpp
#include "vv_common.h"
#include "vv_kernels.h"

namespace {

template <typename T> __device__ __forceinline__ float4 round4_as(float4 a) {
    if constexpr (sizeof(T) == 2) {
        typedef __attribute__((ext_vector_type(4))) float f4v;
        const f4v r = __builtin_convertvector(__builtin_convertvector((f4v){a.x, a.y, a.z, a.w}, bf16x4), f4v);
        return make_float4(r[0], r[1], r[2], r[3]);
    } else {
        return a;
    }
}

template <typename To, typename Td>
__global__ __launch_bounds__(256) void ln_mod_kernel(float* __restrict__ x, int ldx, To* __restrict__ y, int ldy,
                                                     int R, int D, const float* __restrict__ w,
                                                     const float* __restrict__ b, int add_one, float eps,
                                                     const Td* __restrict__ delta, int ldd, const Td* __restrict__ delta2,
                                                     int keep_x, int tail_row0, int tp1, const float* __restrict__ dt1, int tp2,
                                                     const float* __restrict__ dt2) {
    const int lane = threadIdx.x & 63;
    const int row = blockIdx.x * 4 + (threadIdx.x >> 6);
    if (row >= R) return;
    const int n4 = D >> 2;
    float* xr = x + (size_t)row * ldx;
    float4 v[4];
    float s = 0.f;
    if (delta) {
        float4 d[4], d2[4];
        const bool tl1 = tp1 > 0 && row >= tail_row0, tl2 = tp2 > 0 && row >= tail_row0;
        const float4 z4 = make_float4(0.f, 0.f, 0.f, 0.f);
#pragma unroll
        for (int i = 0; i < 4; ++i) {
            const int c = lane + i * 64;
            if (c < n4) {
                v[i] = load4_nt<float>(xr + c * 4);
                d[i] = tl1 ? z4 : load4_nt<Td>(delta + (size_t)row * ldd + c * 4);
                d2[i] = (delta2 && !tl2) ? load4_nt<Td>(delta2 + (size_t)row * ldd + c * 4) : z4;
            } else {
                v[i] = d[i] = d2[i] = z4;
            }
        }
        if (row >= tail_row0) {
            const size_t tr = (size_t)(R - tail_row0), r = (size_t)(row - tail_row0);
            if (tl1) {
                for (int p = 0; p < tp1; ++p)
#pragma unroll
                    for (int i = 0; i < 4; ++i) {
                        const int c = lane + i * 64;
                        if (c < n4) {
                            const float4 t = load4_nt<float>(dt1 + (p * tr + r) * ldd + c * 4);
                            d[i].x += t.x; d[i].y += t.y; d[i].z += t.z; d[i].w += t.w;
                        }
                    }
#pragma unroll
                for (int i = 0; i < 4; ++i) d[i] = round4_as<Td>(d[i]);
            }
            if (tl2) {
                for (int p = 0; p < tp2; ++p)
#pragma unroll
                    for (int i = 0; i < 4; ++i) {
                        const int c = lane + i * 64;
                        if (c < n4) {
                            const float4 t = load4_nt<float>(dt2 + (p * tr + r) * ldd + c * 4);
                            d2[i].x += t.x; d2[i].y += t.y; d2[i].z += t.z; d2[i].w += t.w;
                        }
                    }
#pragma unroll
                for (int i = 0; i < 4; ++i) d2[i] = round4_as<Td>(d2[i]);
            }
        }
#pragma unroll
        for (int i = 0; i < 4; ++i) {
            const int c = lane + i * 64;
            if (c < n4) {
                v[i].x += d[i].x; v[i].y += d[i].y; v[i].z += d[i].z; v[i].w += d[i].w;
                if (delta2) {
                    v[i].x += d2[i].x; v[i].y += d2[i].y; v[i].z += d2[i].z; v[i].w += d2[i].w;
                }
                if (!keep_x) {
                    typedef __attribute__((ext_vector_type(4))) float f4;
                    const f4 w4 = {v[i].x, v[i].y, v[i].z, v[i].w};
                    __builtin_nontemporal_store(w4, (f4*)(xr + c * 4));
                }
                s += (v[i].x + v[i].y) + (v[i].z + v[i].w);
            }
        }
    } else {
#pragma unroll
        for (int i = 0; i < 4; ++i) {
            const int c = lane + i * 64;
            if (c < n4) {
                v[i] = load4_nt<float>(xr + c * 4);
                s += (v[i].x + v[i].y) + (v[i].z + v[i].w);
            } else {
                v[i] = make_float4(0.f, 0.f, 0.f, 0.f);
            }
        }
    }
    const float mean = wave_sum(s) / (float)D;
    float q = 0.f;
#pragma unroll
    for (int i = 0; i < 4; ++i) {
        const int c = lane + i * 64;
        if (c < n4) {
            const float a = v[i].x - mean, bb = v[i].y - mean, cc = v[i].z - mean, dd = v[i].w - mean;
            q += (a * a + bb * bb) + (cc * cc + dd * dd);
        }
    }
    const float rstd = rsqrtf(wave_sum(q) / (float)D + eps);
    const float one = add_one ? 1.0f : 0.0f;
    To* yr = y + (size_t)row * ldy;
#pragma unroll
    for (int i = 0; i < 4; ++i) {
        const int c = lane + i * 64;
        if (c < n4) {
            float4 ww = w ? *(const float4*)(w + c * 4) : make_float4(1.f - one, 1.f - one, 1.f - one, 1.f - one);
            float4 bv = b ? *(const float4*)(b + c * 4) : make_float4(0.f, 0.f, 0.f, 0.f);
            store4<To>(yr + c * 4, (v[i].x - mean) * rstd * (ww.x + one) + bv.x, (v[i].y - mean) * rstd * (ww.y + one) + bv.y,
                       (v[i].z - mean) * rstd * (ww.z + one) + bv.z, (v[i].w - mean) * rstd * (ww.w + one) + bv.w);
        }
    }
}

template <typename T>
__global__ __launch_bounds__(256) void pack_cat_kernel(const float* __restrict__ x, const float* __restrict__ cat,
                                                       const float* __restrict__ cat_drop, T* __restrict__ out, int ldo,
                                                       int BN, int n_mel, int cond_dim, int only_x,
                                                       const int* __restrict__ row_src) {
    const int cols4 = (only_x ? n_mel : ldo) >> 2;
    const size_t total = (size_t)2 * BN * cols4;
    for (size_t i = (size_t)blockIdx.x * 256 + threadIdx.x; i < total; i += (size_t)gridDim.x * 256) {
        const int c = (int)(i % cols4) * 4;
        const size_t row = i / cols4;
        size_t bt = row >= (size_t)BN ? row - BN : row;
        if (row_src) bt = (size_t)row_src[bt];
        float4 v;
        if (c < n_mel) v = *(const float4*)(x + bt * n_mel + c);
        else if (c < n_mel + cond_dim) v = *(const float4*)((row >= (size_t)BN ? cat_drop : cat) + bt * cond_dim + (c - n_mel));
        else v = make_float4(0.f, 0.f, 0.f, 0.f);
        store4<T>(out + row * ldo + c, v.x, v.y, v.z, v.w);
    }
}

template <typename T>
__global__ __launch_bounds__(256) void pack_cat_guided_kernel(const float* __restrict__ x, const float* __restrict__ cat,
                                                              const float* __restrict__ cat_drop, T* __restrict__ out, int ldo, int Rc,
                                                              int row0, int n_rows, int n_mel, int cond_dim, int only_x, int x_packed,
                                                              const int* __restrict__ row_src, const int* __restrict__ u_src,
                                                              const int* __restrict__ u_crow) {
    const int cols4 = (only_x ? n_mel : ldo) >> 2;
    const size_t total = (size_t)n_rows * cols4;
    for (size_t i = (size_t)blockIdx.x * 256 + threadIdx.x; i < total; i += (size_t)gridDim.x * 256) {
        const int c = (int)(i % cols4) * 4;
        const size_t row = (size_t)row0 + i / cols4;
        const bool unc = row >= (size_t)Rc;
        const size_t bt = unc ? (size_t)u_src[row - Rc] : (size_t)row_src[row];
        float4 v;
        if (c < n_mel) v = *(const float4*)(x + (x_packed ? (unc ? (size_t)u_crow[row - Rc] : row) : bt) * n_mel + c);
        else if (c < n_mel + cond_dim) v = *(const float4*)((unc ? cat_drop : cat) + bt * cond_dim + (c - n_mel));
        else v = make_float4(0.f, 0.f, 0.f, 0.f);
        store4<T>(out + row * ldo + c, v.x, v.y, v.z, v.w);
    }
}

__global__ __launch_bounds__(256) void cfg_euler_kernel(float* __restrict__ x, const float* __restrict__ pred, int ldp,
                                                        int BN, int n_mel, float cfg, float dt, const int* __restrict__ row_src) {
    const int c4 = n_mel >> 2;
    const size_t total = (size_t)BN * c4;
    for (size_t i = (size_t)blockIdx.x * 256 + threadIdx.x; i < total; i += (size_t)gridDim.x * 256) {
        const int c = (int)(i % c4) * 4;
        const size_t row = i / c4;
        const float4 pc = *(const float4*)(pred + row * ldp + c);
        const float4 pu = *(const float4*)(pred + (row + BN) * ldp + c);
        const size_t xr = row_src ? (size_t)row_src[row] : row;
        float4 xv = *(float4*)(x + xr * n_mel + c);
        xv.x += dt * (pc.x + (pc.x - pu.x) * cfg);
        xv.y += dt * (pc.y + (pc.y - pu.y) * cfg);
        xv.z += dt * (pc.z + (pc.z - pu.z) * cfg);
        xv.w += dt * (pc.w + (pc.w - pu.w) * cfg);
        *(float4*)(x + xr * n_mel + c) = xv;
    }
}

struct OdeStagePrev { const float* k[3]; float c[3]; };
template <bool GUIDED, bool APG>
__global__ __launch_bounds__(256) void ode_stage_kernel(float* x, const float* __restrict__ pred, int ldp, int BN, int n_mel, float g,
                                                        const float* __restrict__ g_item, int seq_n, const int* __restrict__ row_src,
                                                        OdeStagePrev pv, float c_new, float* __restrict__ k_out, float* __restrict__ x_out,
                                                        const int* __restrict__ u_row, const float* __restrict__ apg_coef,
                                                        const float* x_e, int xe_packed, float omt) {
    const int c4 = n_mel >> 2;
    const size_t total = (size_t)BN * c4;
    for (size_t i = (size_t)blockIdx.x * 256 + threadIdx.x; i < total; i += (size_t)gridDim.x * 256) {
        const int c = (int)(i % c4) * 4;
        const size_t row = i / c4;
        const float4 pc = *(const float4*)(pred + row * ldp + c);
        const size_t xr = row_src ? (size_t)row_src[row] : row;
        float cfg, apg_c = 0.f;
        if (APG) {
            const float2 ac = *(const float2*)(apg_coef + 2 * (xr / (size_t)seq_n));
            cfg = ac.x; apg_c = ac.y;
        } else {
            cfg = g_item ? g_item[xr / (size_t)seq_n] : g;
        }
// ... 299 lines not shown
    __shared__ float red[3][4];
    const int b = blockIdx.y, g = blockIdx.x;
    const int cpg = C / G;
    const size_t n = (size_t)cpg * T;
    const float* xs = x + ((size_t)b * C + (size_t)g * cpg) * T;
    float* ys = y + ((size_t)b * C + (size_t)g * cpg) * T;
    const bool vec = (T & 3) == 0 && (((uintptr_t)xs | (uintptr_t)ys) & 15) == 0;
    const size_t n4 = n >> 2;
    float s0 = 0.f;
    if (vec) {
        for (size_t i = threadIdx.x; i < n4; i += 256) {
            const float4 v = *(const float4*)(xs + i * 4);
            s0 += (v.x + v.y) + (v.z + v.w);
        }
    } else {
        for (size_t i = threadIdx.x; i < n; i += 256) s0 += xs[i];
    }
    s0 = wave_sum(s0);
    if ((threadIdx.x & 63) == 0) red[0][threadIdx.x >> 6] = s0;
    __syncthreads();
    const float m0 = ((red[0][0] + red[0][1]) + (red[0][2] + red[0][3])) / (float)n;
    float s = 0.f, q = 0.f;
    if (vec) {
        for (size_t i = threadIdx.x; i < n4; i += 256) {
            const float4 v = *(const float4*)(xs + i * 4);
            const float a0 = v.x - m0, a1 = v.y - m0, a2 = v.z - m0, a3 = v.w - m0;
            s += (a0 + a1) + (a2 + a3);
            q += (a0 * a0 + a1 * a1) + (a2 * a2 + a3 * a3);
        }
    } else {
        for (size_t i = threadIdx.x; i < n; i += 256) { const float d = xs[i] - m0; s += d; q += d * d; }
    }
    s = wave_sum(s); q = wave_sum(q);
    if ((threadIdx.x & 63) == 0) { red[1][threadIdx.x >> 6] = s; red[2][threadIdx.x >> 6] = q; }
    __syncthreads();
    const float sd = ((red[1][0] + red[1][1]) + (red[1][2] + red[1][3])) / (float)n;
    const float var = fmaxf(((red[2][0] + red[2][1]) + (red[2][2] + red[2][3])) / (float)n - sd * sd, 0.f);
    const float mean = m0 + sd, rstd = rsqrtf(var + eps);
    if (vec) {
        const int t4 = T >> 2;
        for (size_t i = threadIdx.x; i < n4; i += 256) {
            const int c = g * cpg + (int)(i / t4);
            const float ga = (gamma ? gamma[c] : 1.f) * rstd, be = beta ? beta[c] : 0.f;
            const float4 v = *(const float4*)(xs + i * 4);
            float4 o;
            o.x = act_apply((v.x - mean) * ga + be, act); o.y = act_apply((v.y - mean) * ga + be, act);
            o.z = act_apply((v.z - mean) * ga + be, act); o.w = act_apply((v.w - mean) * ga + be, act);
            *(float4*)(ys + i * 4) = o;
        }
    } else {
        for (size_t i = threadIdx.x; i < n; i += 256) {
            const int c = g * cpg + (int)(i / T);
            ys[i] = act_apply((xs[i] - mean) * ((gamma ? gamma[c] : 1.f) * rstd) + (beta ? beta[c] : 0.f), act);
        }
    }
}

__global__ __launch_bounds__(256) void rope_compact_kernel(const float* __restrict__ c, const float* __restrict__ s, float* __restrict__ out, int n) {
    const int i = blockIdx.x * 256 + threadIdx.x;
    if (i >= n * 32) return;
    const int pos = i >> 5, pr = i & 31;
    out[(size_t)pos * 64 + 2 * pr] = c[(size_t)pos * 64 + 2 * pr];
    out[(size_t)pos * 64 + 2 * pr + 1] = s[(size_t)pos * 64 + 2 * pr];
}

__global__ __launch_bounds__(256) void rope_rows_kernel(const float* __restrict__ cs, const int* __restrict__ pos, float* __restrict__ out, int rows) {
    const size_t i = (size_t)blockIdx.x * 256 + threadIdx.x;
    if (i >= (size_t)rows * 16) return;
    const size_t r = i >> 4;
    const int q = (int)(i & 15);
    *(float4*)(out + r * 64 + q * 4) = *(const float4*)(cs + (size_t)pos[r] * 64 + q * 4);
}

inline int grid_for(size_t total) { return (int)std::min<size_t>((total + 255) / 256, 256 * 8); }

}

#define VVK_CHECK_LAUNCH()                                               \
    do {                                                                 \
        hipError_t he__ = hipGetLastError();                             \
        if (he__ != hipSuccess) { *err = hipGetErrorString(he__); return -5; } \
    } while (0)

int vvk_ln_mod(const vv_ln_args* a, hipStream_t st, const char** err) {
    if (a->R <= 0) { *err = "ln: empty"; return -22; }
    if (a->D < 4 || a->D % 4 || a->D > 1024 || a->ldx % 4 || a->ldy % 4) { *err = "ln: D must be a multiple of 4 within [4, 1024]"; return -22; }
    if (a->ldx < a->D || a->ldy < a->D) { *err = "ln: ldx and ldy must be at least D"; return -22; }
    if (a->delta && (a->ld_delta % 4 || a->ld_delta < a->D)) { *err = "ln: bad delta leading dimension"; return -22; }
    if (a->delta2 && !a->delta) { *err = "ln: delta2 without delta"; return -22; }
    const int grid = (a->R + 3) / 4;
    float* x = const_cast<float*>(a->x);
    const bool ob = a->out_dtype == VV_BF16, db = a->delta_dtype == VV_BF16;
    const int tp1 = a->delta && a->delta_tail_parts > 1 ? a->delta_tail_parts : 0, tp2 = a->delta2 && a->delta2_tail_parts > 1 ? a->delta2_tail_parts : 0;
    if ((tp1 || tp2) && (((uintptr_t)a->delta_tail | (uintptr_t)a->delta2_tail) % 16)) { *err = "ln: split-K tail buffers must be 16-byte aligned"; return -22; }
    if ((a->delta_tail_parts > 1 && !a->delta) || (a->delta2_tail_parts > 1 && !a->delta2)) { *err = "ln: a delta tail without its delta"; return -22; }
    if ((tp1 || tp2) && (a->tail_row0 < 0 || a->tail_row0 >= a->R || (tp1 && !a->delta_tail) || (tp2 && !a->delta2_tail) || tp1 > 8 || tp2 > 8)) {
        *err = "ln: bad split-K tail (row0 within [0, R), buffers given, at most 8 parts)"; return -22;
    }
    const int tail_row0 = (tp1 || tp2) ? a->tail_row0 : a->R;
#define LN_GO(To, Td) ln_mod_kernel<To, Td><<<grid, 256, 0, st>>>(x, a->ldx, (To*)a->y, a->ldy, a->R, a->D, a->w, a->b, a->add_one, a->eps, (const Td*)a->delta, a->ld_delta, (const Td*)a->delta2, a->keep_x, tail_row0, tp1, (const float*)a->delta_tail, tp2, (const float*)a->delta2_tail)
    if (ob && db) LN_GO(bf16, bf16);
    else if (ob) LN_GO(bf16, float);
    else if (db) LN_GO(float, bf16);
    else LN_GO(float, float);
#undef LN_GO
    VVK_CHECK_LAUNCH();
    return 0;
}

int vvk_pack_cat(int dtype, const float* x, const float* cat, const float* cat_drop, void* out, int ldo, int BN, int n_mel,
                 int cond_dim, int only_x, const int* row_src, hipStream_t st, const char** err) {
    if (n_mel % 4 || cond_dim % 4 || ldo % 4 || ldo < n_mel + cond_dim) { *err = "pack_cat: bad widths"; return -22; }
    const size_t total = (size_t)2 * BN * ((only_x ? n_mel : ldo) / 4);
    if (dtype == VV_BF16)
        pack_cat_kernel<bf16><<<grid_for(total), 256, 0, st>>>(x, cat, cat_drop, (bf16*)out, ldo, BN, n_mel, cond_dim, only_x, row_src);
    else
        pack_cat_kernel<float><<<grid_for(total), 256, 0, st>>>(x, cat, cat_drop, (float*)out, ldo, BN, n_mel, cond_dim, only_x, row_src);
    VVK_CHECK_LAUNCH();
    return 0;
}

int vvk_cfg_euler(float* x, const float* pred, int ldp, int BN, int n_mel, float cfg, float dt, const int* row_src, hipStream_t st,
                  const char** err) {
    if (n_mel % 4 || ldp % 4) { *err = "cfg_euler: widths must be multiples of 4"; return -22; }
    cfg_euler_kernel<<<grid_for((size_t)BN * n_mel / 4), 256, 0, st>>>(x, pred, ldp, BN, n_mel, cfg, dt, row_src);
    VVK_CHECK_LAUNCH();
    return 0;
}

int vvk_ode_stage(const vv_ode_stage_args* a, const int* u_row, const vv_apg_stage_args* apg, hipStream_t st, const char** err) {
    if (a->n_mel < 4 || a->n_mel % 4 || a->ldp % 4 || a->ldp < a->n_mel || a->Rc < 1) { *err = "ode_stage: widths must be multiples of 4, ldp >= n_mel, Rc >= 1"; return -22; }
    if (!a->x || !a->pred || a->n_prev < 0 || a->n_prev > 3) { *err = "ode_stage: x, pred and 0..3 earlier slopes"; return -22; }
    if (a->g_item && a->seq_n < 1) { *err = "ode_stage: g_item needs the padded sequence length seq_n"; return -22; }
    uintptr_t al = (uintptr_t)a->x | (uintptr_t)a->pred | (uintptr_t)a->k_out | (uintptr_t)a->x_out;
    OdeStagePrev pv{};
    for (int j = 0; j < a->n_prev; ++j) {
        if (!(a->coef[j] == a->coef[j]) || !(a->coef[a->n_prev] == a->coef[a->n_prev])) { *err = "ode_stage: NaN coefficient"; return -22; }
        if (a->coef[j] == 0.f) continue;
        if (!a->k_prev[j]) { *err = "ode_stage: a non-zero coefficient without its slope buffer"; return -22; }
        pv.k[j] = a->k_prev[j]; pv.c[j] = a->coef[j];
        al |= (uintptr_t)a->k_prev[j];
        if (a->k_prev[j] == a->k_out || a->k_prev[j] == a->x_out) { *err = "ode_stage: an output aliases an earlier slope"; return -22; }
    }
    if (al % 16) { *err = "ode_stage: buffers must be 16-byte aligned"; return -22; }
    if (a->x_out && (a->x_out == a->x || a->x_out == a->k_out)) { *err = "ode_stage: x_out must be a buffer of its own"; return -22; }
    if (apg) {
        if (!apg->coef || !apg->x_e || a->seq_n < 1) { *err = "ode_stage: APG needs coef, x_e and the padded sequence length seq_n"; return -22; }
        if (((uintptr_t)apg->coef % 8) || ((uintptr_t)apg->x_e % 16)) { *err = "ode_stage: APG coef must be 8-byte and x_e 16-byte aligned"; return -22; }
        if (apg->x_e == a->x_out || apg->x_e == a->k_out) { *err = "ode_stage: APG x_e aliases an output of the launch"; return -22; }
        if (!(apg->t_e == apg->t_e)) { *err = "ode_stage: NaN evaluation time"; return -22; }
    }
    const int grid = grid_for((size_t)a->Rc * a->n_mel / 4);
    const float omt = apg ? 1.0f - apg->t_e : 0.f;
#define STAGE_GO(G, A) ode_stage_kernel<G, A><<<grid, 256, 0, st>>>(a->x, a->pred, a->ldp, a->Rc, a->n_mel, a->g, a->g_item, a->seq_n, a->row_src, pv, \
        a->coef[a->n_prev], a->k_out, a->x_out, u_row, apg ? apg->coef : nullptr, apg ? apg->x_e : nullptr, apg ? apg->x_e_packed : 0, omt)
    if (apg) { if (u_row) STAGE_GO(true, true); else STAGE_GO(false, true); }
    else if (u_row) STAGE_GO(true, false);
    else STAGE_GO(false, false);
#undef STAGE_GO
    VVK_CHECK_LAUNCH();
    return 0;
}

int vvk_apg_coef(const vv_apg_coef_args* a, int which, hipStream_t st, const char** err) {
    if (a->n_mel < 4 || a->n_mel % 4 || a->ldp % 4 || a->ldp < a->n_mel || a->Rc < 1) { *err = "apg_coef: widths must be multiples of 4, ldp >= n_mel, Rc >= 1"; return -22; }
    if (!a->pred || !a->x_e || !a->row_start || !a->len || !a->partials || !a->coef) { *err = "apg_coef: pred, x_e, row_start, len, partials and coef are required"; return -22; }
    if (a->B < 1 || a->B > VVK_GUIDE_MAX_ITEMS || a->n_tiles < 1) { *err = "apg_coef: 1..1024 items, n_tiles >= 1"; return -22; }
    if (((uintptr_t)a->pred | (uintptr_t)a->x_e) % 16 || (uintptr_t)a->partials % 8 || (uintptr_t)a->coef % 8) { *err = "apg_coef: pred and x_e 16-byte, partials and coef 8-byte aligned"; return -22; }
    if (!(a->t_e == a->t_e)) { *err = "apg_coef: NaN evaluation time"; return -22; }
    const double omt = 1.0 - (double)a->t_e;
    if (which & 1) {
        apg_reduce_kernel<<<dim3(a->n_tiles, a->B), 256, 0, st>>>(a->pred, a->ldp, a->Rc, a->n_mel, a->u_row, a->x_e, a->row_src, a->row_start,
                                                                   a->len, a->n_tiles, omt, a->partials);
        VVK_CHECK_LAUNCH();
    }
    if (which & 2) {
        apg_coef_kernel<<<a->B, 64, 0, st>>>(a->partials, a->n_tiles, a->Rc, a->n_mel, a->u_row, a->row_start, a->len, omt, a->g, a->g_item,
                                             a->eta, a->norm_rms, a->coef);
        VVK_CHECK_LAUNCH();
    }
    return 0;
}

// ... 114 lines not shown
```

### vietvoice-tts_amd/csrc/vv_kernels.h

```cpp
#pragma once
#include <hip/hip_runtime.h>
#include <algorithm>
#include "../../include/vvtts.h"

typedef vv_gemm_args vvk_gemm_args;

int vvk_gemm(const vv_gemm_args* g, hipStream_t st, const char** err);
void vvk_gemm_tail_plan(int M, int N, int K, int lda, int ldw, int ldc, int* row0, int* parts);
int vvk_attention(const vv_attn_args* a, hipStream_t st, const char** err);
int vvk_ln_mod(const vv_ln_args* a, hipStream_t st, const char** err);
int vvk_posconv(const vv_posconv_args* a, hipStream_t st, const char** err);
int vvk_conv(const vv_conv_args* a, hipStream_t st, const char** err);
int vvk_conv_x3(const vv_conv_args* a, hipStream_t st, const char** err);
size_t vvk_conv_split_bytes(int Cin_pad, int KW, int rows_pad);
int vvk_conv_split_weights(const float* Wt, int Cin_pad, int KW, int rows_pad, void* Wb, hipStream_t st, const char** err);
int vvk_mrf_pair(const vv_mrf_args* a, hipStream_t st, const char** err);
int vvk_conv_post(const float* in, const float* w, float bias, int16_t* pcm, int ld_pcm, float* wave_f32, int B, int C, int T,
                  int KW, float pre_slope, const int* len_in, hipStream_t st, const char** err);
int vvk_mel_slice(const float* x, int B, int N, int n_mel, const int* ref_len, const int* seq_len, float* out, int T,
                  hipStream_t st, const char** err);
int vvk_mel(const int16_t* audio, int ld_audio, const int* audio_len, const float* window, const float* tw_cos,
            const float* tw_sin, const float* fb, float* mel, int B, int F_max, int n_fft, int hop, int n_mel, hipStream_t st,
            const char** err);
int vvk_pack_cat(int dtype, const float* x, const float* cat, const float* cat_drop, void* out, int ldo, int BN, int n_mel,
                 int cond_dim, int only_x, const int* row_src, hipStream_t st, const char** err);
int vvk_cfg_euler(float* x, const float* pred, int ldp, int BN, int n_mel, float cfg, float dt, const int* row_src, hipStream_t st,
                  const char** err);
int vvk_ode_stage(const vv_ode_stage_args* a, const int* u_row, const vv_apg_stage_args* apg, hipStream_t st, const char** err);
int vvk_apg_coef(const vv_apg_coef_args* a, int which, hipStream_t st, const char** err);
#define VVK_GUIDE_MAX_ITEMS 1024
int vvk_guided_tables(const int* seq_len, const unsigned char* flags, int B, int N, int Rc, int Ru, int* row_start, int* rs_rel, int* kv_len,
                      int* row_pos, int* u_src, int* u_crow, int* u_row, hipStream_t st, const char** err);
int vvk_pack_cat_guided(int dtype, const float* x, const float* cat, const float* cat_drop, void* out, int ldo, int Rc, int row0, int n_rows,
                        int n_mel, int cond_dim, int only_x, int x_packed, const int* row_src, const int* u_src, const int* u_crow,
                        hipStream_t st, const char** err);
int vvk_text_embed(const int* ids, int ld_ids, const int* text_len, const float* emb, const float* pos, float* out, int B, int N,
                   int Dt, int vocab_rows, hipStream_t st, const char** err);
int vvk_dwconv(const float* in, float* out, const float* w, const float* bias, const int* seq_len, int B, int n_seq, int N, int C,
               int KW, hipStream_t st, const char** err);
int vvk_grn(int dtype, void* x, float* sumsq, const float* gamma, const float* beta, const int* seq_len, int B, int n_seq, int N,
            int C, hipStream_t st, const char** err);
int vvk_build_cat(const float* mel, int F_max, const int* ref_len, const float* text, float* cat, float* cat_drop, int B, int N,
                  int n_mel, int Dt, hipStream_t st, const char** err, const uint8_t* keep = nullptr, int ld_keep = 0);
int vvk_ref_len(const int* audio_len, int* ref_len, int B, int hop, hipStream_t st, const char** err);
int vvk_decode_len(const int* seq_len, const int* ref_len, int* lens, int B, int n_levels, const int* mult, hipStream_t st,
                   const char** err);
int vvk_row_tables(const int* seq_len, int B, int N, int Rc, int* row_start, int* row_src, int* row_pos, int* kv_len, hipStream_t st, const char** err);
int vvk_resample_poly(const float* x, int n_in, const double* h, int n_taps, int up, int down, int skip, float* y, int n_out,
                      hipStream_t st, const char** err);
int vvk_ingest_pcm(const void* pcm, const long long* desc, int n_clips, long long max_out, float* out, hipStream_t st, const char** err);
size_t vvk_normalize_scratch_bytes(int n_clips, long long total_len);
int vvk_normalize_clips(const float* x, const long long* off, int n_clips, long long max_len, void* scratch, int16_t* out,
                        hipStream_t st, const char** err);
int vvk_rope_compact(const float* c, const float* s, float* out, int n, hipStream_t st, const char** err);
int vvk_rope_rows(const float* cs, const int* pos, float* out, int rows, hipStream_t st, const char** err);
int vvk_groupnorm(const float* x, float* y, const float* gamma, const float* beta, int B, int C, int T, int G, float eps, int act,
                  hipStream_t st, const char** err);
int vvk_edit_splice(const int16_t* src, long long n_src, const long long* desc, int n_rows, int B, int16_t* out, int ld_out,
                    hipStream_t st, const char** err);
int vvk_edit_restore(float* x, const float* cat, const uint8_t* keep, int ld_keep, const int* seq_len, int B, int N, int n_mel, int cd,
                     hipStream_t st, const char** err);
int vvk_noise_fill(float* x, const int* seq_len, const unsigned long long* keys, int B, int N, int n_mel, int kind, hipStream_t st,
                   const char** err);
int vvk_join_max_n();
int vvk_join_chunks(const int16_t* pcm, long long n_pcm, const long long* chunk_rows, int n_chunks, const long long* req_rows, int R,
                    const double* fade, long long n_fade, int max_n, long long max_len, int16_t* out, long long n_out, void* ws,
                    hipStream_t st, const char** err);
int vvk_pcm_resample(const int16_t* x, long long n_x, const long long* rows, int n_rows, long long max_out, const double* taps, int n_taps,
                     int up, int down, int skip, int16_t* y, long long n_y, hipStream_t st, const char** err);
int vvk_pcm_encode(const int16_t* x, long long n_x, const long long* rows, int n_rows, long long max_n, int kind, uint8_t* y, long long n_y,
                   hipStream_t st, const char** err);
unsigned long long vvk_pcm_loudness_ws_bytes(long long total_runs, int R);
int vvk_pcm_loudness(const int16_t* x, long long n_x, const long long* rows, int R, long long sub, long long total_runs, long long max_n,
                     const double* tables, const double* params, int16_t* y, long long n_y, double* stats, void* ws, hipStream_t st,
                     const char** err);
int vvk_pcm_limit_tile(int L);
unsigned long long vvk_pcm_limit_ws_bytes(long long total_samples, long long total_tiles, int R);
int vvk_pcm_limit(const int16_t* x, long long n_x, const long long* rows, int R, int L, int mode, long long total_samples,
                  long long total_tiles, long long max_tiles, long long max_out, const double* window, const double* taps,
                  const double* params, const double* meas, int16_t* y, long long n_y, double* stats, void* ws, hipStream_t st,
                  const char** err);
unsigned long long vvk_pcm_stretch_ws_bytes(int R);
int vvk_pcm_stretch(const int16_t* x, long long n_x, const long long* rows, int R, long long max_out, const double* window, int16_t* y,
                    long long n_y, int* pos, long long n_pos, void* ws, hipStream_t st, const char** err);
unsigned long long vvk_flac_frame_bound(long long m);
unsigned long long vvk_pcm_flac_ws_bytes(long long total_frames, int R);
unsigned long long vvk_pcm_flac_lpc_ws_bytes(long long total_frames, int R);
int vvk_pcm_flac(const int16_t* x, long long n_x, const long long* rows, int R, int rate, int lpc_order, long long total_frames, long long max_frames,
                 uint8_t* y, long long n_y, long long* info, void* ws, hipStream_t st, const char** err);
int vvk_vocos_lens(const int* seq_len, const int* ref_len, int* lens, int B, int N, int T_max, hipStream_t st, const char** err);
int vvk_vocos_im2col(const float* x, int B, int N, int M, const int* ref_len, const int* seq_len, int T_max, int k, float* out, int ld_out,
                     hipStream_t st, const char** err);
int vvk_vocos_spectrum(const float* head, int ld_head, int R, int n_fft, float* out, hipStream_t st, const char** err);
// ... 3 lines not shown
```

### vietvoice-tts_amd/runtime.py

```python
from __future__ import annotations

import ctypes as C
import os
import contextlib
import threading
from typing import Dict, Optional, Tuple

import torch

from . import pack
from .model_spec import ODE_MAX_EVALS, ModelSpec, check_apg, guidance_mask, ode_plan

_HERE = os.path.dirname(os.path.abspath(__file__))
LIB_PATH = os.environ.get("VVTTS_LIB") or os.path.join(_HERE, "libvvtts_hip.so")

VV_F32, VV_BF16 = 0, 1
PROF_CLASSES = ["gemm", "attention", "norm", "posconv", "elementwise", "voc_conv", "voc_post", "mel", "text",
                "voc_pre", "voc_up0", "voc_up1", "voc_up2", "voc_up3", "voc_mrf0", "voc_mrf1", "voc_mrf2", "voc_mrf3"]


class HipUnavailable(RuntimeError):
    pass


# ... 55 lines not shown
                ("KW", C.c_int32), ("dil", C.c_int32), ("transposed", C.c_int32), ("up", C.c_int32),
                ("rows_total", C.c_int32), ("rows_pad", C.c_int32), ("accumulate", C.c_int32),
                ("pre_slope", C.c_float), ("out_scale", C.c_float), ("len_in", C.c_void_p), ("W_x3", C.c_void_p), ("wg_rows", C.c_int32)]


class vv_mrf_args(C.Structure):
    _fields_ = [("y", C.c_void_p), ("W1", C.c_void_p), ("b1", C.c_void_p), ("W2", C.c_void_p), ("b2", C.c_void_p), ("out", C.c_void_p),
                ("B", C.c_int32), ("C", C.c_int32), ("T", C.c_int32), ("KW", C.c_int32), ("dil", C.c_int32), ("rows_pad", C.c_int32),
                ("accumulate", C.c_int32), ("slope", C.c_float), ("out_scale", C.c_float), ("len_in", C.c_void_p)]


class vv_steps_args(C.Structure):
    _fields_ = [("B", C.c_int32), ("N", C.c_int32), ("seq_len", C.c_void_p), ("seq_len_host", C.c_void_p), ("x", C.c_void_p),
                ("cat_mel_text", C.c_void_p), ("cat_mel_text_drop", C.c_void_p), ("rope_cos_q", C.c_void_p), ("rope_sin_q", C.c_void_p),
                ("rope_cos_k", C.c_void_p), ("rope_sin_k", C.c_void_p), ("step0", C.c_int32), ("n_steps", C.c_int32),
                ("ws", C.c_void_p), ("ws_bytes", C.c_uint64), ("cfg_item", C.c_void_p)]


class vv_ode_stage_args(C.Structure):
    _fields_ = [("x", C.c_void_p), ("pred", C.c_void_p), ("ldp", C.c_int32), ("Rc", C.c_int32), ("n_mel", C.c_int32), ("n_prev", C.c_int32),
                ("k_prev", C.c_void_p * 3), ("coef", C.c_float * 4), ("k_out", C.c_void_p), ("x_out", C.c_void_p),
                ("g", C.c_float), ("g_item", C.c_void_p), ("seq_n", C.c_int32), ("row_src", C.c_void_p)]


class vv_apg_args(C.Structure):
    _fields_ = [("eta", C.c_void_p), ("norm_rms", C.c_void_p), ("t_host", C.c_void_p)]


class vv_apg_coef_args(C.Structure):
    _fields_ = [("pred", C.c_void_p), ("ldp", C.c_int32), ("Rc", C.c_int32), ("n_mel", C.c_int32), ("u_row", C.c_void_p),
                ("x_e", C.c_void_p), ("row_src", C.c_void_p), ("B", C.c_int32), ("n_tiles", C.c_int32), ("row_start", C.c_void_p),
                ("len", C.c_void_p), ("t_e", C.c_float), ("g", C.c_float), ("g_item", C.c_void_p), ("eta", C.c_void_p),
                ("norm_rms", C.c_void_p), ("partials", C.c_void_p), ("coef", C.c_void_p)]


class vv_apg_stage_args(C.Structure):
    _fields_ = [("coef", C.c_void_p), ("x_e", C.c_void_p), ("x_e_packed", C.c_int32), ("t_e", C.c_float)]


APG_TILE = 32

EXPORTS = {
    "vv_version": (C.c_char_p, []),
    "vv_last_error": (C.c_char_p, [C.c_void_p]),
    "vv_create": (C.c_int, [C.POINTER(C.c_void_p), C.c_int, C.POINTER(vv_model_cfg), C.c_int]),
    "vv_destroy": (None, [C.c_void_p]),
    "vv_bind_weight": (C.c_int, [C.c_void_p, C.c_char_p, C.c_void_p, C.c_uint64]),
    "vv_finalize_weights": (C.c_int, [C.c_void_p]),
    "vv_set_time_grid": (C.c_int, [C.c_void_p, C.c_void_p, C.c_void_p, C.c_int, C.c_void_p]),
    "vv_set_ode_plan": (C.c_int, [C.c_void_p, C.c_void_p, C.c_void_p, C.c_int, C.c_int, C.c_void_p, C.c_void_p, C.c_void_p]),
    "vv_transformer_steps_ex": (C.c_int, [C.c_void_p, C.POINTER(vv_steps_args), C.c_void_p]),
    "vv_ode_stage": (C.c_int, [C.c_void_p, C.POINTER(vv_ode_stage_args), C.c_void_p]),
    "vv_transformer_steps_guided": (C.c_int, [C.c_void_p, C.POINTER(vv_steps_args), C.c_void_p, C.c_int, C.c_void_p]),
    "vv_transformer_guided_ws_bytes": (C.c_int, [C.c_void_p, C.c_int, C.c_int, C.c_void_p, C.POINTER(C.c_uint64)]),
    "vv_ode_stage_guided": (C.c_int, [C.c_void_p, C.POINTER(vv_ode_stage_args), C.c_void_p, C.c_void_p]),
    "vv_transformer_steps_apg": (C.c_int, [C.c_void_p, C.POINTER(vv_steps_args), C.c_void_p, C.c_int, C.POINTER(vv_apg_args), C.c_void_p]),
    "vv_transformer_apg_ws_bytes": (C.c_int, [C.c_void_p, C.c_int, C.c_int, C.c_void_p, C.POINTER(C.c_uint64)]),
    "vv_apg_coef": (C.c_int, [C.c_void_p, C.POINTER(vv_apg_coef_args), C.c_void_p]),
    "vv_ode_stage_apg": (C.c_int, [C.c_void_p, C.POINTER(vv_ode_stage_args), C.c_void_p, C.POINTER(vv_apg_stage_args), C.c_void_p]),
    "vv_preprocess": (C.c_int, [C.c_void_p, C.c_int, C.c_int, C.c_void_p, C.c_int, C.c_int, C.c_void_p, C.c_void_p, C.c_int,
                                C.c_void_p, C.c_void_p, C.c_void_p, C.c_void_p, C.c_void_p, C.c_void_p]),
    "vv_preprocess_h": (C.c_int, [C.c_void_p, C.c_int, C.c_int, C.c_void_p, C.c_int, C.c_int, C.c_void_p, C.c_void_p, C.c_void_p, C.c_int,
                                  C.c_void_p, C.c_void_p, C.c_void_p, C.c_void_p, C.c_void_p, C.c_void_p]),
    "vv_transformer_steps": (C.c_int, [C.c_void_p, C.c_int, C.c_int, C.c_void_p, C.c_void_p, C.c_void_p, C.c_void_p, C.c_void_p,
                                       C.c_void_p, C.c_void_p, C.c_void_p, C.c_int, C.c_int, C.c_void_p]),
    "vv_transformer_steps_h": (C.c_int, [C.c_void_p, C.c_int, C.c_int, C.c_void_p, C.c_void_p, C.c_void_p, C.c_void_p, C.c_void_p, C.c_void_p,
                                         C.c_void_p, C.c_void_p, C.c_void_p, C.c_int, C.c_int, C.c_void_p]),
    "vv_transformer_ws_bytes": (C.c_int, [C.c_void_p, C.c_int, C.c_int, C.c_void_p, C.POINTER(C.c_uint64)]),
    "vv_transformer_steps_into": (C.c_int, [C.c_void_p, C.c_int, C.c_int, C.c_void_p, C.c_void_p, C.c_void_p, C.c_void_p, C.c_void_p, C.c_void_p,
                                            C.c_void_p, C.c_void_p, C.c_void_p, C.c_int, C.c_int, C.c_void_p, C.c_uint64, C.c_void_p]),
    "vv_decode": (C.c_int, [C.c_void_p, C.c_int, C.c_int, C.c_void_p, C.c_void_p, C.c_void_p, C.c_int, C.c_void_p, C.c_int,
                            C.c_void_p, C.c_void_p, C.c_void_p]),
    "vv_decode_ws_bytes": (C.c_int, [C.c_void_p, C.c_int, C.c_int, C.POINTER(C.c_uint64)]),
    "vv_decode_into": (C.c_int, [C.c_void_p, C.c_int, C.c_int, C.c_void_p, C.c_void_p, C.c_void_p, C.c_int, C.c_void_p, C.c_int,
                                 C.c_void_p, C.c_void_p, C.c_void_p, C.c_uint64, C.c_void_p]),
    "vv_ws_generation": (C.c_uint64, [C.c_void_p]),
    "vv_set_option": (C.c_int, [C.c_void_p, C.c_char_p, C.c_int]),
    "vv_set_rope_theta": (C.c_int, [C.c_void_p, C.c_float]),
    "vv_prof_enable": (C.c_int, [C.c_void_p, C.c_int]),
    "vv_prof_collect": (C.c_int, [C.c_void_p, C.c_void_p, C.c_void_p, C.c_void_p, C.c_void_p]),
    "vv_gemm": (C.c_int, [C.c_void_p, C.POINTER(vv_gemm_args), C.c_void_p]),
    "vv_attention": (C.c_int, [C.c_void_p, C.POINTER(vv_attn_args), C.c_void_p]),
    "vv_layernorm": (C.c_int, [C.c_void_p, C.POINTER(vv_ln_args), C.c_void_p]),
    "vv_posconv": (C.c_int, [C.c_void_p, C.POINTER(vv_posconv_args), C.c_void_p]),
    "vv_conv1d": (C.c_int, [C.c_void_p, C.POINTER(vv_conv_args), C.c_void_p]),
    "vv_mrf_resblock": (C.c_int, [C.c_void_p, C.POINTER(vv_mrf_args), C.c_void_p]),
    "vv_conv_post": (C.c_int, [C.c_void_p, C.c_void_p, C.c_void_p, C.c_float, C.c_void_p, C.c_int, C.c_void_p, C.c_int, C.c_int,
                               C.c_int, C.c_int, C.c_float, C.c_void_p, C.c_void_p]),
    "vv_mel": (C.c_int, [C.c_void_p, C.c_void_p, C.c_int, C.c_void_p, C.c_void_p, C.c_int, C.c_int, C.c_void_p]),
    "vv_groupnorm": (C.c_int, [C.c_void_p, C.c_void_p, C.c_void_p, C.c_void_p, C.c_void_p, C.c_int, C.c_int, C.c_int, C.c_int, C.c_float,
                               C.c_int, C.c_void_p]),
    "vv_text_embed": (C.c_int, [C.c_void_p, C.c_void_p, C.c_int, C.c_void_p, C.c_void_p, C.c_void_p, C.c_int, C.c_void_p, C.c_int, C.c_int, C.c_int,
                                C.c_void_p]),
    "vv_dwconv": (C.c_int, [C.c_void_p, C.c_void_p, C.c_void_p, C.c_void_p, C.c_void_p, C.c_void_p, C.c_int, C.c_int, C.c_int, C.c_int, C.c_int,
                            C.c_void_p]),
    "vv_grn": (C.c_int, [C.c_void_p, C.c_int, C.c_void_p, C.c_void_p, C.c_void_p, C.c_void_p, C.c_void_p, C.c_int, C.c_int, C.c_int, C.c_int,
                         C.c_void_p]),
    "vv_rope_compact": (C.c_int, [C.c_void_p, C.c_void_p, C.c_void_p, C.c_void_p, C.c_int, C.c_void_p]),
    "vv_conv_split_bytes": (C.c_uint64, [C.c_int32, C.c_int32, C.c_int32]),
    "vv_conv_split_weights": (C.c_int, [C.c_void_p, C.c_void_p, C.c_int32, C.c_int32, C.c_int32, C.c_void_p, C.c_void_p]),
    "vv_gemm_tail_plan": (C.c_int, [C.c_void_p, C.c_int32, C.c_int32, C.c_int32, C.POINTER(C.c_int32), C.POINTER(C.c_int32)]),
    "vv_rope_rows": (C.c_int, [C.c_void_p, C.c_void_p, C.c_void_p, C.c_void_p, C.c_int, C.c_void_p]),
    "vv_cfg_euler": (C.c_int, [C.c_void_p, C.c_void_p, C.c_void_p, C.c_int, C.c_int, C.c_int, C.c_float, C.c_float, C.c_void_p]),
    "vv_resample_poly": (C.c_int, [C.c_void_p, C.c_void_p, C.c_int, C.c_void_p, C.c_int, C.c_int, C.c_int, C.c_int, C.c_void_p, C.c_int, C.c_void_p]),
    "vv_ingest_pcm": (C.c_int, [C.c_void_p, C.c_void_p, C.c_void_p, C.c_int, C.c_int64, C.c_void_p, C.c_void_p]),
    "vv_normalize_scratch_bytes": (C.c_size_t, [C.c_int, C.c_int64]),
    "vv_normalize_clips": (C.c_int, [C.c_void_p, C.c_void_p, C.c_void_p, C.c_int, C.c_int64, C.c_void_p, C.c_void_p, C.c_void_p]),
    "vv_edit_splice": (C.c_int, [C.c_void_p, C.c_void_p, C.c_int64, C.c_void_p, C.c_int, C.c_int, C.c_void_p, C.c_int, C.c_void_p]),
    "vv_preprocess_edit": (C.c_int, [C.c_void_p, C.c_int, C.c_int, C.c_void_p, C.c_int, C.c_int, C.c_void_p, C.c_void_p, C.c_void_p, C.c_int,
                                     C.c_void_p, C.c_void_p, C.c_void_p, C.c_void_p, C.c_void_p, C.c_void_p, C.c_int, C.c_void_p]),
    "vv_noise_fill": (C.c_int, [C.c_void_p, C.c_int, C.c_int, C.c_int, C.c_void_p, C.c_void_p, C.c_void_p, C.c_int, C.c_void_p]),
    "vv_edit_restore": (C.c_int, [C.c_void_p, C.c_int, C.c_int, C.c_void_p, C.c_void_p, C.c_void_p, C.c_int, C.c_void_p, C.c_void_p]),
    "vv_join_chunks": (C.c_int, [C.c_void_p, C.c_void_p, C.c_int64, C.c_void_p, C.c_void_p, C.c_int, C.c_void_p, C.c_void_p, C.c_int, C.c_void_p,
                                 C.c_int64, C.c_int, C.c_int64, C.c_void_p, C.c_int64, C.c_void_p, C.c_void_p]),
    "vv_pcm_resample": (C.c_int, [C.c_void_p, C.c_void_p, C.c_int64, C.c_void_p, C.c_int, C.c_int64, C.c_void_p, C.c_int, C.c_int, C.c_int,
                                  C.c_int, C.c_void_p, C.c_int64, C.c_void_p]),
    "vv_pcm_encode": (C.c_int, [C.c_void_p, C.c_void_p, C.c_int64, C.c_void_p, C.c_int, C.c_int64, C.c_int, C.c_void_p, C.c_int64, C.c_void_p]),
    "vv_pcm_loudness_ws_bytes": (C.c_uint64, [C.c_int64, C.c_int]),
    "vv_pcm_loudness": (C.c_int, [C.c_void_p, C.c_void_p, C.c_int64, C.c_void_p, C.c_void_p, C.c_int, C.c_int64, C.c_void_p, C.c_void_p, C.c_void_p,
                                  C.c_int64, C.c_void_p, C.c_void_p, C.c_uint64, C.c_void_p]),
    "vv_pcm_limit_tile": (C.c_int, [C.c_int]),
    "vv_pcm_limit_ws_bytes": (C.c_uint64, [C.c_int64, C.c_int64, C.c_int]),
    "vv_pcm_limit": (C.c_int, [C.c_void_p, C.c_void_p, C.c_int64, C.c_void_p, C.c_void_p, C.c_int, C.c_int, C.c_int, C.c_void_p, C.c_void_p,
                               C.c_void_p, C.c_void_p, C.c_void_p, C.c_int64, C.c_void_p, C.c_void_p, C.c_uint64, C.c_void_p]),
    "vv_flac_frame_bound": (C.c_uint64, [C.c_int64]),
    "vv_pcm_flac_ws_bytes": (C.c_uint64, [C.c_int64, C.c_int]),
    "vv_pcm_flac_lpc_ws_bytes": (C.c_uint64, [C.c_int64, C.c_int, C.c_int]),
    "vv_pcm_flac_lpc": (C.c_int, [C.c_void_p, C.c_void_p, C.c_int64, C.c_void_p, C.c_void_p, C.c_int, C.c_int, C.c_int, C.c_void_p, C.c_int64,
                                  C.c_void_p, C.c_void_p, C.c_uint64, C.c_void_p]),
    "vv_pcm_flac": (C.c_int, [C.c_void_p, C.c_void_p, C.c_int64, C.c_void_p, C.c_void_p, C.c_int, C.c_int, C.c_void_p, C.c_int64, C.c_void_p,
                              C.c_void_p, C.c_uint64, C.c_void_p]),
    "vv_pcm_stretch_ws_bytes": (C.c_uint64, [C.c_int]),
    "vv_pcm_stretch": (C.c_int, [C.c_void_p, C.c_void_p, C.c_int64, C.c_void_p, C.c_void_p, C.c_int, C.c_void_p, C.c_void_p, C.c_int64, C.c_void_p,
                                 C.c_int64, C.c_void_p, C.c_uint64, C.c_void_p]),
    "vv_set_vocos": (C.c_int, [C.c_void_p, C.POINTER(vv_vocos_cfg)]),
    "vv_vocos_im2col": (C.c_int, [C.c_void_p, C.c_void_p, C.c_int, C.c_int, C.c_void_p, C.c_void_p, C.c_int, C.c_void_p, C.c_int, C.c_void_p]),
    "vv_istft_head": (C.c_int, [C.c_void_p, C.c_int, C.c_int, C.c_void_p, C.c_int, C.c_void_p, C.c_void_p, C.c_int, C.c_void_p, C.c_void_p,
                                C.c_void_p]),
}

_lib = None
_lib_lock = threading.Lock()


def load_library(path: Optional[str] = None):
    global _lib
    with _lib_lock:
        if _lib is not None and path is None:
            return _lib
        p = path or LIB_PATH
        if not os.path.exists(p):
            raise HipUnavailable(f"{p} not found: build it with `python __graft_entry__.py` (hipcc --offload-arch=gfx950); "
                                 "the HIP synthesis path has no CPU fallback")
        lib = C.CDLL(p)
        for name, (res, args) in EXPORTS.items():
            fn = getattr(lib, name)
            fn.restype, fn.argtypes = res, args
        if path is None:
            _lib = lib
        return lib


def cfg_from_spec(spec: ModelSpec) -> vv_model_cfg:
    c = vv_model_cfg()
    c.n_mel, c.n_fft, c.win_length, c.hop_length = spec.n_mel, spec.n_fft, spec.win_length, spec.hop_length
    c.dim, c.depth, c.heads, c.head_dim, c.ff_mult = spec.dim, spec.depth, spec.heads, spec.head_dim, spec.ff_mult
# ... 1150 lines not shown
```

Before: 194.6.

## Fuse each lane's first LayerNorm into the other lane's attention kernel

When two lanes run in parallel (bf16, no split-K tails), the pre-attention modulated LayerNorm for one lane is appended as a rider to the tail of the other lane's attention kernel. This removes one LayerNorm launch per block per lane. It also interleaves the two lanes' blocks with cross-stream events so each rider's inputs are ready. It adds cross-lane synchronisation that can reduce the independent overlap between lanes, and it lengthens the attention kernel with row-wise norm work.

```diff
diff --git a/include/vvtts.h b/include/vvtts.h
--- a/include/vvtts.h
+++ b/include/vvtts.h
@@ -209,6 +209,7 @@
     const void *delta_tail, *delta2_tail;
 } vv_ln_args;
 VV_API int vv_layernorm(vv_ctx* ctx, const vv_ln_args* args, void* stream);
+VV_API int vv_attention_ln(vv_ctx* ctx, const vv_attn_args* attn_args, const vv_ln_args* ln_args, void* stream);
 
 typedef struct vv_posconv_args {
     int32_t dtype, out_dtype;
diff --git a/vietvoice-tts_amd/csrc/vv_api.hip b/vietvoice-tts_amd/csrc/vv_api.hip
--- a/vietvoice-tts_amd/csrc/vv_api.hip
+++ b/vietvoice-tts_amd/csrc/vv_api.hip
@@ -55,6 +55,8 @@
     int lanes = 0;
     hipStream_t side_stream[1] = {};
     hipEvent_t ev_fork = nullptr, ev_join[1] = {};
+    int ln_rider = 1;
+    hipEvent_t ev_att[2] = {}, ev_ready[2] = {};
     float rope_theta = 0.f;
     int rope_q_attn = 1;
     int voc_x3 = -1;
@@ -219,6 +221,8 @@
     for (auto q : c->side_stream) if (q) hipStreamDestroy(q);
     if (c->ev_fork) hipEventDestroy(c->ev_fork);
     for (auto e : c->ev_join) if (e) hipEventDestroy(e);
+    for (auto e : c->ev_att) if (e) hipEventDestroy(e);
+    for (auto e : c->ev_ready) if (e) hipEventDestroy(e);
     for (auto& r : c->recs) { hipEventDestroy(r.a); hipEventDestroy(r.b); }
     for (auto e : c->pool) hipEventDestroy(e);
     delete c;
@@ -1022,7 +1026,25 @@
         L.pending = false;
         return 0;
     };
-    auto block = [&](Lane& L, int s, int l) -> int {
+    auto ln1_args = [&](const Lane& L, int s, int l) -> vv_ln_args {
+        const bool pending = L.pending, tail = l == g.depth;
+        vv_ln_args a{}; a.out_dtype = c->dt; a.x = L.xres; a.ldx = D; a.y = L.h; a.ldy = D; a.R = (int)L.R; a.D = D; a.add_one = 1; a.eps = 1e-6f;
+        a.delta_dtype = c->dt; a.ld_delta = D;
+        a.tail_row0 = L.tail_row0; a.delta_tail = L.h2_tail; a.delta2_tail = L.h3_tail;
+        a.delta_tail_parts = pending ? L.tp_o : 0; a.delta2_tail_parts = pending ? L.tp_f : 0;
+        if (tail) {
+            const float* fm = c->fintab + (size_t)s * 2 * D;
+            a.w = fm; a.b = fm + D;
+        } else {
+            const float* mod = c->modtab + ((size_t)l * S + s) * 6 * D;
+            a.w = mod + D; a.b = mod;
+        }
+        a.delta = pending ? L.h2 : nullptr; a.delta2 = pending ? L.h3 : nullptr;
+        a.keep_x = tail ? 1 : 0;
+        return a;
+    };
+    enum { P_LN1 = 1, P_QKV = 2, P_ATT = 4, P_REST = 8, P_ALL = 15 };
+    auto block = [&](Lane& L, int s, int l, int parts = P_ALL, const vv_ln_args* rider = nullptr) -> int {
         hipStream_t st = L.st;
         const size_t R = L.R;
         const bool pending = L.pending;
@@ -1030,26 +1052,24 @@
         const std::string qkvw = blk(l, ".attn.qkv.weight"), qkvb = blk(l, ".attn.qkv.bias"), ow = blk(l, ".attn.out.weight"),
                           ob = blk(l, ".attn.out.bias"), f1w = blk(l, ".ff1.weight"), f1b = blk(l, ".ff1.bias"),
                           f2w = blk(l, ".ff2.weight"), f2b = blk(l, ".ff2.bias");
-        vv_ln_args a{}; a.out_dtype = c->dt; a.x = L.xres; a.ldx = D; a.y = L.h; a.ldy = D; a.R = (int)R; a.D = D; a.add_one = 1; a.eps = 1e-6f;
-        a.delta_dtype = c->dt; a.ld_delta = D;
-        a.tail_row0 = L.tail_row0; a.delta_tail = L.h2_tail; a.delta2_tail = L.h3_tail;
-        a.delta_tail_parts = pending ? L.tp_o : 0; a.delta2_tail_parts = pending ? L.tp_f : 0;
-        a.w = mod + D; a.b = mod;
-        a.delta = pending ? L.h2 : nullptr; a.delta2 = pending ? L.h3 : nullptr; a.keep_x = 0;
-        { Prof p(c, VV_PROF_NORM, 0, (4.0 + es) * R * D + (pending ? (4.0 + 2.0 * es) * R * D : 0), st); KCHK(c, vvk_ln_mod(&a, st, &m__)); }
-        Gemm qkv = gemm_args(c, c->dt, c->dt, VV_EPI_QKV_ROPE, VV_ACT_NONE_, L.h, D, qkvw.c_str(), D, qkvb.c_str(), L.qkv, 3 * D, (int)R, 3 * D, D);
-        qkv.cos_q = rope_cos_q; qkv.sin_q = rope_sin_q; qkv.cos_k = rope_cos_k; qkv.sin_k = rope_sin_k;
-        qkv.rope_cs_q = c->rope_rows ? L.csq_rows : L.csq; qkv.rope_cs_k = c->rope_rows ? L.csk_rows : L.csk; qkv.rope_by_row = c->rope_rows;
-        qkv.seq_n = N; qkv.rope_dim = D; qkv.rope_pos = L.qkv_pos; qkv.rope_skip_q = q_rope_attn; qkv.rope_theta = rope_theta;
-        if (int r = launch_gemm(c, qkv, VV_PROF_GEMM, st)) return r;
-        {
+        vv_ln_args a = ln1_args(L, s, l);
+        if (parts & P_LN1) { Prof p(c, VV_PROF_NORM, 0, (4.0 + es) * R * D + (pending ? (4.0 + 2.0 * es) * R * D : 0), st); KCHK(c, vvk_ln_mod(&a, st, &m__)); }
+        if (parts & P_QKV) {
+            Gemm qkv = gemm_args(c, c->dt, c->dt, VV_EPI_QKV_ROPE, VV_ACT_NONE_, L.h, D, qkvw.c_str(), D, qkvb.c_str(), L.qkv, 3 * D, (int)R, 3 * D, D);
+            qkv.cos_q = rope_cos_q; qkv.sin_q = rope_sin_q; qkv.cos_k = rope_cos_k; qkv.sin_k = rope_sin_k;
+            qkv.rope_cs_q = c->rope_rows ? L.csq_rows : L.csq; qkv.rope_cs_k = c->rope_rows ? L.csk_rows : L.csk; qkv.rope_by_row = c->rope_rows;
+            qkv.seq_n = N; qkv.rope_dim = D; qkv.rope_pos = L.qkv_pos; qkv.rope_skip_q = q_rope_attn; qkv.rope_theta = rope_theta;
+            if (int r = launch_gemm(c, qkv, VV_PROF_GEMM, st)) return r;
+        }
+        if (parts & P_ATT) {
             vv_attn_args t{}; t.dtype = c->dt; t.qkv = L.qkv; t.ld_qkv = 3 * D; t.out = L.att; t.ld_out = D; t.n_seq = L.n_seq; t.seq_n = N;
             t.heads = g.heads; t.dim = D; t.kv_len = L.kv_len; t.row_start = L.row_start; t.total_rows = (int)R;
             t.rope_cs_q = q_rope_attn ? L.csq : nullptr;
             t.q_scale = rope_theta > 0.f ? 1.0f / sqrtf((float)g.head_dim) : 0.f;
             Prof p(c, VV_PROF_ATTN, 4.0 * g.heads * L.sum_sq * 64, (double)es * R * 4 * D, st);
-            KCHK(c, vvk_attention(&t, st, &m__));
-        }
+            KCHK(c, rider ? vvk_attention_ln(&t, rider, st, &m__) : vvk_attention(&t, st, &m__));
+        }
+        if (!(parts & P_REST)) return 0;
         Gemm out = gemm_args(c, c->dt, c->dt, VV_EPI_GATE_STORE, VV_ACT_NONE_, L.att, D, ow.c_str(), D, ob.c_str(), L.h2, D, (int)R, D, D);
         out.gate = mod + 2 * D;
         if (L.tp_o) { out.C_tail = L.h2_tail; out.tail_row0 = L.tail_row0; out.tail_parts = L.tp_o; }
@@ -1065,18 +1085,12 @@
         L.pending = true;
         return 0;
     };
-    auto step_tail = [&](Lane& L, int s) -> int {
+    auto step_tail = [&](Lane& L, int s, bool with_norm = true) -> int {
         hipStream_t st = L.st;
         const size_t R = L.R;
         const bool pending = L.pending;
-        {
-            const float* fm = c->fintab + (size_t)s * 2 * D;
-            vv_ln_args a{}; a.out_dtype = c->dt; a.x = L.xres; a.ldx = D; a.y = L.h; a.ldy = D; a.R = (int)R; a.D = D; a.add_one = 1; a.eps = 1e-6f;
-            a.w = fm; a.b = fm + D;
-            a.delta = pending ? L.h2 : nullptr; a.delta2 = pending ? L.h3 : nullptr; a.keep_x = 1;
-            a.delta_dtype = c->dt; a.ld_delta = D;
-            a.tail_row0 = L.tail_row0; a.delta_tail = L.h2_tail; a.delta2_tail = L.h3_tail;
-            a.delta_tail_parts = pending ? L.tp_o : 0; a.delta2_tail_parts = pending ? L.tp_f : 0;
+        if (with_norm) {
+            vv_ln_args a = ln1_args(L, s, g.depth);
             Prof p(c, VV_PROF_NORM, 0, es * R * D + (pending ? (4.0 + 2.0 * es) * R * D : 4.0 * R * D), st);
             KCHK(c, vvk_ln_mod(&a, st, &m__));
         }
@@ -1173,6 +1187,41 @@
         hipEventRecord(c->ev_join[0], c->side_stream[0]);
         hipStreamWaitEvent(st, c->ev_join[0], 0);
     };
+    bool tails = false;
+    for (int li = 0; li < n_lanes; ++li) tails = tails || lanes[li].tp_o || lanes[li].tp_f;
+    const bool ride_plan = c->ln_rider && n_lanes == 2 && c->dt == VV_DTYPE_BF16 && !tails && g.depth >= 1;
+    if (ride_plan)
+        for (int i = 0; i < 2; ++i) {
+            if (!c->ev_att[i]) HIPCHK(c, hipEventCreateWithFlags(&c->ev_att[i], hipEventDisableTiming));
+            if (!c->ev_ready[i]) HIPCHK(c, hipEventCreateWithFlags(&c->ev_ready[i], hipEventDisableTiming));
+        }
+    auto eval_ride = [&](int e) -> int {
+        Lane &A = views[0], &Bv = views[1];
+        for (int v = 0; v < 2; ++v) if (int r = step_head(views[v], e)) return r;
+        if (int r = block(A, e, 0, P_LN1)) return r;
+        HIPCHK(c, hipEventRecord(c->ev_ready[1], Bv.st));
+        for (int l = 0; l < g.depth; ++l) {
+            if (l > 0) HIPCHK(c, hipStreamWaitEvent(A.st, c->ev_att[1], 0));
+            if (int r = block(A, e, l, P_QKV)) return r;
+            HIPCHK(c, hipStreamWaitEvent(A.st, c->ev_ready[1], 0));
+            const vv_ln_args rb = ln1_args(Bv, e, l);
+            if (int r = block(A, e, l, P_ATT, &rb)) return r;
+            HIPCHK(c, hipEventRecord(c->ev_att[0], A.st));
+            if (int r = block(A, e, l, P_REST)) return r;
+            HIPCHK(c, hipEventRecord(c->ev_ready[0], A.st));
+            HIPCHK(c, hipStreamWaitEvent(Bv.st, c->ev_att[0], 0));
+            if (int r = block(Bv, e, l, P_QKV)) return r;
+            HIPCHK(c, hipStreamWaitEvent(Bv.st, c->ev_ready[0], 0));
+            const vv_ln_args ra = ln1_args(A, e, l + 1);
+            if (int r = block(Bv, e, l, P_ATT, &ra)) return r;
+            HIPCHK(c, hipEventRecord(c->ev_att[1], Bv.st));
+            if (int r = block(Bv, e, l, P_REST)) return r;
+            HIPCHK(c, hipEventRecord(c->ev_ready[1], Bv.st));
+        }
+        HIPCHK(c, hipStreamWaitEvent(A.st, c->ev_att[1], 0));
+        if (int r = step_tail(A, e, false)) return r;
+        return step_tail(Bv, e);
+    };
     int rc = 0;
     c->chip_share = n_views;
     if (n_lanes > 1) rc = fork();
@@ -1190,10 +1239,14 @@
             const bool want_fork = branch_lanes && n_views == 2;
             if (want_fork && !rc) rc = fork();
             const bool forked = want_fork && !rc;
-            for (int v = 0; v < n_views && !rc; ++v) rc = step_head(views[v], e);
-            for (int l = 0; l < g.depth && !rc; ++l)
-                for (int v = 0; v < n_views && !rc; ++v) rc = block(views[v], e, l);
-            for (int v = 0; v < n_views && !rc; ++v) rc = step_tail(views[v], e);
+            if (ride_plan && n_views == 2 && views[0].R > 0 && views[1].R > 0) {
+                if (!rc) rc = eval_ride(e);
+            } else {
+                for (int v = 0; v < n_views && !rc; ++v) rc = step_head(views[v], e);
+                for (int l = 0; l < g.depth && !rc; ++l)
+                    for (int v = 0; v < n_views && !rc; ++v) rc = block(views[v], e, l);
+                for (int v = 0; v < n_views && !rc; ++v) rc = step_tail(views[v], e);
+            }
             if (forked) join();
             for (int li = 0; li < n_lanes && !rc; ++li) rc = rk ? step_stage(lanes[li], s, i) : step_euler(lanes[li], s);
         }
@@ -1506,6 +1559,10 @@
         if (value < 0 || value > 2) return c->fail(-22, "vv_set_option: lanes takes 0 (auto), 1 (one lane) or 2 (two lanes whenever the batch has two items)");
         c->lanes = value; return 0;
     }
+    if (!strcmp(name, "ln_rider")) {
+        if (value < 0 || value > 1) return c->fail(-22, "vv_set_option: ln_rider takes 0 (every LayerNorm a launch of its own) or 1 (first norms ride in the other lane's attention)");
+        c->ln_rider = value; return 0;
+    }
     if (!strcmp(name, "fuse_mrf")) {
         if (value < 0 || value > 2) return c->fail(-22, "vv_set_option: fuse_mrf takes 0 (off), 1 (on) or 2 (auto)");
         c->fuse_mrf = value; return 0;
@@ -1569,6 +1626,7 @@
 }
 int vv_attention(vv_ctx* c, const vv_attn_args* a, void* st) { SINGLE(c, vvk_attention(a, (hipStream_t)st, &m__)); }
 int vv_layernorm(vv_ctx* c, const vv_ln_args* a, void* st) { SINGLE(c, vvk_ln_mod(a, (hipStream_t)st, &m__)); }
+int vv_attention_ln(vv_ctx* c, const vv_attn_args* a, const vv_ln_args* ln, void* st) { SINGLE(c, vvk_attention_ln(a, ln, (hipStream_t)st, &m__)); }
 int vv_posconv(vv_ctx* c, const vv_posconv_args* a, void* st) { SINGLE(c, vvk_posconv(a, (hipStream_t)st, &m__)); }
 int vv_conv1d(vv_ctx* c, const vv_conv_args* a, void* st) { SINGLE(c, vvk_conv(a, (hipStream_t)st, &m__)); }
 uint64_t vv_conv_split_bytes(int32_t Cin_pad, int32_t KW, int32_t rows_pad) {
diff --git a/vietvoice-tts_amd/csrc/vv_attention.hip b/vietvoice-tts_amd/csrc/vv_attention.hip
--- a/vietvoice-tts_amd/csrc/vv_attention.hip
+++ b/vietvoice-tts_amd/csrc/vv_attention.hip
@@ -1,5 +1,6 @@
 #include "vv_common.h"
 #include "vv_kernels.h"
+#include "vv_ln_row.h"
 
 namespace {
 
@@ -64,16 +65,15 @@
 #define VV_ATTN_ABLATE 0
 #endif
 
-__global__ __launch_bounds__(256, 2) void attn_bf16_kernel(const bf16* __restrict__ qkv, int ld, bf16* __restrict__ out,
-                                                           int ldo, int seq_n, int D, const int* __restrict__ kv_len_arr,
-                                                           const int* __restrict__ row_start, int total_rows, int heads, int n_seq,
-                                                           const float* __restrict__ rope_cs_q, float q_mul) {
+__device__ __forceinline__ void attn_bf16_block(const bf16* __restrict__ qkv, int ld, bf16* __restrict__ out,
+                                                int ldo, int seq_n, int D, const int* __restrict__ kv_len_arr,
+                                                const int* __restrict__ row_start, int total_rows, int heads, int n_seq,
+                                                const float* __restrict__ rope_cs_q, float q_mul, const int wave) {
     __shared__ __attribute__((aligned(16))) char smem[2 * 16384];
     const AttnBlock blk = attn_block((seq_n + 127) / 128, heads, n_seq);
     if (!blk.valid) return;
     const int head = blk.head, seq = blk.seq, qblock = blk.qb;
     const int lane = threadIdx.x & 63;
-    const int wave = __builtin_amdgcn_readfirstlane(threadIdx.x >> 6);
     const int r32 = lane & 31, h = lane >> 5;
     int kv_len = kv_len_arr ? kv_len_arr[seq] : seq_n;
     if (row_start && kv_len <= 0) return;
@@ -303,6 +303,23 @@
     }
 }
 
+__global__ __launch_bounds__(256, 2) void attn_bf16_kernel(const bf16* __restrict__ qkv, int ld, bf16* __restrict__ out,
+                                                           int ldo, int seq_n, int D, const int* __restrict__ kv_len_arr,
+                                                           const int* __restrict__ row_start, int total_rows, int heads, int n_seq,
+                                                           const float* __restrict__ rope_cs_q, float q_mul, LnRowArgs ln, int R_ln) {
+    const int wave = __builtin_amdgcn_readfirstlane(threadIdx.x >> 6);
+    attn_bf16_block(qkv, ld, out, ldo, seq_n, D, kv_len_arr, row_start, total_rows, heads, n_seq, rope_cs_q, q_mul, wave);
+    if (ln.x == nullptr) return;
+    const long long G = gridDim.x, j = blockIdx.x;
+    int r0 = (int)(j * R_ln / G), r1 = (int)((j + 1) * R_ln / G);
+    asm volatile("" : "+s"(r0), "+s"(r1));
+    const int lane = (int)__builtin_amdgcn_mbcnt_hi(~0u, __builtin_amdgcn_mbcnt_lo(~0u, 0u));
+    ln.tp1 = ln.tp2 = 0;
+    ln.tail_row0 = ln.R;
+#pragma nounroll
+    for (int row = r0 + wave; row < r1; row += 4) ln_row<bf16, bf16>(row, lane, ln);
+}
+
 __global__ __launch_bounds__(256, 2) void attn_f32_kernel(const float* __restrict__ qkv, int ld, float* __restrict__ out,
                                                           int ldo, int seq_n, int D, const int* __restrict__ kv_len_arr,
                                                           const int* __restrict__ row_start, int heads, int n_seq) {
@@ -439,7 +456,7 @@
 
 }
 
-int vvk_attention(const vv_attn_args* a, hipStream_t st, const char** err) {
+static int attention_launch(const vv_attn_args* a, const LnRowArgs* ln, hipStream_t st, const char** err) {
     if (a->n_seq <= 0 || a->seq_n <= 0 || a->heads <= 0) { *err = "attention: empty shape"; return -22; }
     if (a->dim != a->heads * 64) { *err = "attention: head_dim must be 64"; return -22; }
     const int esz = a->dtype == VV_BF16 ? 2 : 4;
@@ -459,7 +476,8 @@
     const dim3 grid((unsigned)(pairs8 * nqb * 8));
     if (a->dtype == VV_BF16)
         attn_bf16_kernel<<<grid, 256, 0, st>>>((const bf16*)a->qkv, a->ld_qkv, (bf16*)a->out, a->ld_out, a->seq_n, a->dim, a->kv_len, a->row_start, total_rows,
-                                               a->heads, a->n_seq, a->rope_cs_q, LOG2E * (a->q_scale > 0.f ? a->q_scale : 1.0f));
+                                               a->heads, a->n_seq, a->rope_cs_q, LOG2E * (a->q_scale > 0.f ? a->q_scale : 1.0f), ln ? *ln : LnRowArgs{},
+                                               ln ? ln->R : 0);
     else
         attn_f32_kernel<<<grid, 256, 0, st>>>((const float*)a->qkv, a->ld_qkv, (float*)a->out, a->ld_out, a->seq_n, a->dim, a->kv_len, a->row_start,
                                               a->heads, a->n_seq);
@@ -467,3 +485,19 @@
     if (he != hipSuccess) { *err = hipGetErrorString(he); return -5; }
     return 0;
 }
+
+int vvk_attention(const vv_attn_args* a, hipStream_t st, const char** err) { return attention_launch(a, nullptr, st, err); }
+
+int vvk_attention_ln(const vv_attn_args* a, const vv_ln_args* ln, hipStream_t st, const char** err) {
+    if (!ln || !ln->x || ln->R == 0) return attention_launch(a, nullptr, st, err);
+    if (a->dtype != VV_BF16) { *err = "attention_ln: the rider is the bf16 kernel's"; return -22; }
+    if (ln->out_dtype != VV_BF16 || ((ln->delta || ln->delta2) && ln->delta_dtype != VV_BF16)) { *err = "attention_ln: the rider takes bf16 deltas and writes a bf16 norm"; return -22; }
+    LnRowArgs k;
+    const int rc = vvk_ln_check(ln, &k, err);
+    if (rc) return rc;
+    if (k.tp1 || k.tp2) { *err = "attention_ln: the rider takes no split-K tail (launch the norm on its own)"; return -22; }
+    if (((uintptr_t)ln->x | (uintptr_t)ln->w | (uintptr_t)ln->b) % 16 || ((uintptr_t)ln->y | (uintptr_t)ln->delta | (uintptr_t)ln->delta2) % 8) {
+        *err = "attention_ln: x, w, b must be 16-byte aligned, y and the deltas 8-byte aligned"; return -22;
+    }
+    return attention_launch(a, &k, st, err);
+}
diff --git a/vietvoice-tts_amd/csrc/vv_elementwise.hip b/vietvoice-tts_amd/csrc/vv_elementwise.hip
--- a/vietvoice-tts_amd/csrc/vv_elementwise.hip
+++ b/vietvoice-tts_amd/csrc/vv_elementwise.hip
@@ -1,17 +1,8 @@
 #include "vv_common.h"
 #include "vv_kernels.h"
+#include "vv_ln_row.h"
 
 namespace {
-
-template <typename T> __device__ __forceinline__ float4 round4_as(float4 a) {
-    if constexpr (sizeof(T) == 2) {
-        typedef __attribute__((ext_vector_type(4))) float f4v;
-        const f4v r = __builtin_convertvector(__builtin_convertvector((f4v){a.x, a.y, a.z, a.w}, bf16x4), f4v);
-        return make_float4(r[0], r[1], r[2], r[3]);
-    } else {
-        return a;
-    }
-}
 
 template <typename To, typename Td>
 __global__ __launch_bounds__(256) void ln_mod_kernel(float* __restrict__ x, int ldx, To* __restrict__ y, int ldy,
@@ -23,105 +14,7 @@
     const int lane = threadIdx.x & 63;
     const int row = blockIdx.x * 4 + (threadIdx.x >> 6);
     if (row >= R) return;
-    const int n4 = D >> 2;
-    float* xr = x + (size_t)row * ldx;
-    float4 v[4];
-    float s = 0.f;
-    if (delta) {
-        float4 d[4], d2[4];
-        const bool tl1 = tp1 > 0 && row >= tail_row0, tl2 = tp2 > 0 && row >= tail_row0;
-        const float4 z4 = make_float4(0.f, 0.f, 0.f, 0.f);
-#pragma unroll
-        for (int i = 0; i < 4; ++i) {
-            const int c = lane + i * 64;
-            if (c < n4) {
-                v[i] = load4_nt<float>(xr + c * 4);
-                d[i] = tl1 ? z4 : load4_nt<Td>(delta + (size_t)row * ldd + c * 4);
-                d2[i] = (delta2 && !tl2) ? load4_nt<Td>(delta2 + (size_t)row * ldd + c * 4) : z4;
-            } else {
-                v[i] = d[i] = d2[i] = z4;
-            }
-        }
-        if (row >= tail_row0) {
-            const size_t tr = (size_t)(R - tail_row0), r = (size_t)(row - tail_row0);
-            if (tl1) {
-                for (int p = 0; p < tp1; ++p)
-#pragma unroll
-                    for (int i = 0; i < 4; ++i) {
-                        const int c = lane + i * 64;
-                        if (c < n4) {
-                            const float4 t = load4_nt<float>(dt1 + (p * tr + r) * ldd + c * 4);
-                            d[i].x += t.x; d[i].y += t.y; d[i].z += t.z; d[i].w += t.w;
-                        }
-                    }
-#pragma unroll
-                for (int i = 0; i < 4; ++i) d[i] = round4_as<Td>(d[i]);
-            }
-            if (tl2) {
-                for (int p = 0; p < tp2; ++p)
-#pragma unroll
-                    for (int i = 0; i < 4; ++i) {
-                        const int c = lane + i * 64;
-                        if (c < n4) {
-                            const float4 t = load4_nt<float>(dt2 + (p * tr + r) * ldd + c * 4);
-                            d2[i].x += t.x; d2[i].y += t.y; d2[i].z += t.z; d2[i].w += t.w;
-                        }
-                    }
-#pragma unroll
-                for (int i = 0; i < 4; ++i) d2[i] = round4_as<Td>(d2[i]);
-            }
-        }
-#pragma unroll
-        for (int i = 0; i < 4; ++i) {
-            const int c = lane + i * 64;
-            if (c < n4) {
-                v[i].x += d[i].x; v[i].y += d[i].y; v[i].z += d[i].z; v[i].w += d[i].w;
-                if (delta2) {
-                    v[i].x += d2[i].x; v[i].y += d2[i].y; v[i].z += d2[i].z; v[i].w += d2[i].w;
-                }
-                if (!keep_x) {
-                    typedef __attribute__((ext_vector_type(4))) float f4;
-                    const f4 w4 = {v[i].x, v[i].y, v[i].z, v[i].w};
-                    __builtin_nontemporal_store(w4, (f4*)(xr + c * 4));
-                }
-                s += (v[i].x + v[i].y) + (v[i].z + v[i].w);
-            }
-        }
-    } else {
-#pragma unroll
-        for (int i = 0; i < 4; ++i) {
-            const int c = lane + i * 64;
-            if (c < n4) {
-                v[i] = load4_nt<float>(xr + c * 4);
-                s += (v[i].x + v[i].y) + (v[i].z + v[i].w);
-            } else {
-                v[i] = make_float4(0.f, 0.f, 0.f, 0.f);
-            }
-        }
-    }
-    const float mean = wave_sum(s) / (float)D;
-    float q = 0.f;
-#pragma unroll
-    for (int i = 0; i < 4; ++i) {
-        const int c = lane + i * 64;
-        if (c < n4) {
-            const float a = v[i].x - mean, bb = v[i].y - mean, cc = v[i].z - mean, dd = v[i].w - mean;
-            q += (a * a + bb * bb) + (cc * cc + dd * dd);
-        }
-    }
-    const float rstd = rsqrtf(wave_sum(q) / (float)D + eps);
-    const float one = add_one ? 1.0f : 0.0f;
-    To* yr = y + (size_t)row * ldy;
-#pragma unroll
-    for (int i = 0; i < 4; ++i) {
-        const int c = lane + i * 64;
-        if (c < n4) {
-            float4 ww = w ? *(const float4*)(w + c * 4) : make_float4(1.f - one, 1.f - one, 1.f - one, 1.f - one);
-            float4 bv = b ? *(const float4*)(b + c * 4) : make_float4(0.f, 0.f, 0.f, 0.f);
-            store4<To>(yr + c * 4, (v[i].x - mean) * rstd * (ww.x + one) + bv.x, (v[i].y - mean) * rstd * (ww.y + one) + bv.y,
-                       (v[i].z - mean) * rstd * (ww.z + one) + bv.z, (v[i].w - mean) * rstd * (ww.w + one) + bv.w);
-        }
-    }
+    ln_row<To, Td>(row, lane, x, ldx, y, ldy, R, D, w, b, add_one, eps, delta, ldd, delta2, keep_x, tail_row0, tp1, dt1, tp2, dt2);
 }
 
 template <typename T>
@@ -587,23 +480,30 @@
         if (he__ != hipSuccess) { *err = hipGetErrorString(he__); return -5; } \
     } while (0)
 
-int vvk_ln_mod(const vv_ln_args* a, hipStream_t st, const char** err) {
+int vvk_ln_check(const vv_ln_args* a, LnRowArgs* k, const char** err) {
     if (a->R <= 0) { *err = "ln: empty"; return -22; }
     if (a->D < 4 || a->D % 4 || a->D > 1024 || a->ldx % 4 || a->ldy % 4) { *err = "ln: D must be a multiple of 4 within [4, 1024]"; return -22; }
     if (a->ldx < a->D || a->ldy < a->D) { *err = "ln: ldx and ldy must be at least D"; return -22; }
     if (a->delta && (a->ld_delta % 4 || a->ld_delta < a->D)) { *err = "ln: bad delta leading dimension"; return -22; }
     if (a->delta2 && !a->delta) { *err = "ln: delta2 without delta"; return -22; }
-    const int grid = (a->R + 3) / 4;
-    float* x = const_cast<float*>(a->x);
-    const bool ob = a->out_dtype == VV_BF16, db = a->delta_dtype == VV_BF16;
     const int tp1 = a->delta && a->delta_tail_parts > 1 ? a->delta_tail_parts : 0, tp2 = a->delta2 && a->delta2_tail_parts > 1 ? a->delta2_tail_parts : 0;
     if ((tp1 || tp2) && (((uintptr_t)a->delta_tail | (uintptr_t)a->delta2_tail) % 16)) { *err = "ln: split-K tail buffers must be 16-byte aligned"; return -22; }
     if ((a->delta_tail_parts > 1 && !a->delta) || (a->delta2_tail_parts > 1 && !a->delta2)) { *err = "ln: a delta tail without its delta"; return -22; }
     if ((tp1 || tp2) && (a->tail_row0 < 0 || a->tail_row0 >= a->R || (tp1 && !a->delta_tail) || (tp2 && !a->delta2_tail) || tp1 > 8 || tp2 > 8)) {
         *err = "ln: bad split-K tail (row0 within [0, R), buffers given, at most 8 parts)"; return -22;
     }
-    const int tail_row0 = (tp1 || tp2) ? a->tail_row0 : a->R;
-#define LN_GO(To, Td) ln_mod_kernel<To, Td><<<grid, 256, 0, st>>>(x, a->ldx, (To*)a->y, a->ldy, a->R, a->D, a->w, a->b, a->add_one, a->eps, (const Td*)a->delta, a->ld_delta, (const Td*)a->delta2, a->keep_x, tail_row0, tp1, (const float*)a->delta_tail, tp2, (const float*)a->delta2_tail)
+    *k = LnRowArgs{const_cast<float*>(a->x), a->ldx, a->y, a->ldy, a->R, a->D, a->w, a->b, a->add_one, a->eps, a->delta, a->ld_delta, a->delta2,
+                   a->keep_x, (tp1 || tp2) ? a->tail_row0 : a->R, tp1, (const float*)a->delta_tail, tp2, (const float*)a->delta2_tail};
+    return 0;
+}
+
+int vvk_ln_mod(const vv_ln_args* a, hipStream_t st, const char** err) {
+    LnRowArgs k;
+    const int rc = vvk_ln_check(a, &k, err);
+    if (rc) return rc;
+    const int grid = (a->R + 3) / 4;
+    const bool ob = a->out_dtype == VV_BF16, db = a->delta_dtype == VV_BF16;
+#define LN_GO(To, Td) ln_mod_kernel<To, Td><<<grid, 256, 0, st>>>(k.x, k.ldx, (To*)k.y, k.ldy, k.R, k.D, k.w, k.b, k.add_one, k.eps, (const Td*)k.delta, k.ldd, (const Td*)k.delta2, k.keep_x, k.tail_row0, k.tp1, k.dt1, k.tp2, k.dt2)
     if (ob && db) LN_GO(bf16, bf16);
     else if (ob) LN_GO(bf16, float);
     else if (db) LN_GO(float, bf16);
diff --git a/vietvoice-tts_amd/csrc/vv_kernels.h b/vietvoice-tts_amd/csrc/vv_kernels.h
--- a/vietvoice-tts_amd/csrc/vv_kernels.h
+++ b/vietvoice-tts_amd/csrc/vv_kernels.h
@@ -9,6 +9,9 @@
 void vvk_gemm_tail_plan(int M, int N, int K, int lda, int ldw, int ldc, int* row0, int* parts);
 int vvk_attention(const vv_attn_args* a, hipStream_t st, const char** err);
 int vvk_ln_mod(const vv_ln_args* a, hipStream_t st, const char** err);
+struct LnRowArgs;
+int vvk_ln_check(const vv_ln_args* a, LnRowArgs* k, const char** err);
+int vvk_attention_ln(const vv_attn_args* a, const vv_ln_args* ln, hipStream_t st, const char** err);
 int vvk_posconv(const vv_posconv_args* a, hipStream_t st, const char** err);
 int vvk_conv(const vv_conv_args* a, hipStream_t st, const char** err);
 int vvk_conv_x3(const vv_conv_args* a, hipStream_t st, const char** err);
diff --git a/vietvoice-tts_amd/csrc/vv_ln_row.h b/vietvoice-tts_amd/csrc/vv_ln_row.h
--- /dev/null
+++ b/vietvoice-tts_amd/csrc/vv_ln_row.h
@@ -0,0 +1,140 @@
+#pragma once
+#include "vv_common.h"
+
+template <typename T> __device__ __forceinline__ float4 round4_as(float4 a) {
+    if constexpr (sizeof(T) == 2) {
+        typedef __attribute__((ext_vector_type(4))) float f4v;
+        const f4v r = __builtin_convertvector(__builtin_convertvector((f4v){a.x, a.y, a.z, a.w}, bf16x4), f4v);
+        return make_float4(r[0], r[1], r[2], r[3]);
+    } else {
+        return a;
+    }
+}
+
+struct LnRowArgs {
+    float* x; int ldx;
+    void* y; int ldy;
+    int R, D;
+    const float* w; const float* b;
+    int add_one; float eps;
+    const void* delta; int ldd;
+    const void* delta2;
+    int keep_x;
+    int tail_row0, tp1;
+    const float* dt1;
+    int tp2;
+    const float* dt2;
+};
+
+template <typename To, typename Td>
+__device__ __forceinline__ void ln_row(const int row, const int lane, float* __restrict__ x, const int ldx, To* __restrict__ y, const int ldy,
+                                       const int R, const int D, const float* __restrict__ w, const float* __restrict__ b, const int add_one,
+                                       const float eps, const Td* __restrict__ delta, const int ldd, const Td* __restrict__ delta2,
+                                       const int keep_x, const int tail_row0, const int tp1, const float* __restrict__ dt1, const int tp2,
+                                       const float* __restrict__ dt2) {
+    const int n4 = D >> 2;
+    float* xr = x + (size_t)row * ldx;
+    float4 v[4];
+    float s = 0.f;
+    if (delta) {
+        float4 d[4], d2[4];
+        const bool tl1 = tp1 > 0 && row >= tail_row0, tl2 = tp2 > 0 && row >= tail_row0;
+        const float4 z4 = make_float4(0.f, 0.f, 0.f, 0.f);
+#pragma unroll
+        for (int i = 0; i < 4; ++i) {
+            const int c = lane + i * 64;
+            if (c < n4) {
+                v[i] = load4_nt<float>(xr + c * 4);
+                d[i] = tl1 ? z4 : load4_nt<Td>(delta + (size_t)row * ldd + c * 4);
+                d2[i] = (delta2 && !tl2) ? load4_nt<Td>(delta2 + (size_t)row * ldd + c * 4) : z4;
+            } else {
+                v[i] = d[i] = d2[i] = z4;
+            }
+        }
+        if (row >= tail_row0) {
+            const size_t tr = (size_t)(R - tail_row0), r = (size_t)(row - tail_row0);
+            if (tl1) {
+                for (int p = 0; p < tp1; ++p)
+#pragma unroll
+                    for (int i = 0; i < 4; ++i) {
+                        const int c = lane + i * 64;
+                        if (c < n4) {
+                            const float4 t = load4_nt<float>(dt1 + (p * tr + r) * ldd + c * 4);
+                            d[i].x += t.x; d[i].y += t.y; d[i].z += t.z; d[i].w += t.w;
+                        }
+                    }
+#pragma unroll
+                for (int i = 0; i < 4; ++i) d[i] = round4_as<Td>(d[i]);
+            }
+            if (tl2) {
+                for (int p = 0; p < tp2; ++p)
+#pragma unroll
+                    for (int i = 0; i < 4; ++i) {
+                        const int c = lane + i * 64;
+                        if (c < n4) {
+                            const float4 t = load4_nt<float>(dt2 + (p * tr + r) * ldd + c * 4);
+                            d2[i].x += t.x; d2[i].y += t.y; d2[i].z += t.z; d2[i].w += t.w;
+                        }
+                    }
+#pragma unroll
+                for (int i = 0; i < 4; ++i) d2[i] = round4_as<Td>(d2[i]);
+            }
+        }
+#pragma unroll
+        for (int i = 0; i < 4; ++i) {
+            const int c = lane + i * 64;
+            if (c < n4) {
+                v[i].x += d[i].x; v[i].y += d[i].y; v[i].z += d[i].z; v[i].w += d[i].w;
+                if (delta2) {
+                    v[i].x += d2[i].x; v[i].y += d2[i].y; v[i].z += d2[i].z; v[i].w += d2[i].w;
+                }
+                if (!keep_x) {
+                    typedef __attribute__((ext_vector_type(4))) float f4;
+                    const f4 w4 = {v[i].x, v[i].y, v[i].z, v[i].w};
+                    __builtin_nontemporal_store(w4, (f4*)(xr + c * 4));
+                }
+                s += (v[i].x + v[i].y) + (v[i].z + v[i].w);
+            }
+        }
+    } else {
+#pragma unroll
+        for (int i = 0; i < 4; ++i) {
+            const int c = lane + i * 64;
+            if (c < n4) {
+                v[i] = load4_nt<float>(xr + c * 4);
+                s += (v[i].x + v[i].y) + (v[i].z + v[i].w);
+            } else {
+                v[i] = make_float4(0.f, 0.f, 0.f, 0.f);
+            }
+        }
+    }
+    const float mean = wave_sum(s) / (float)D;
+    float q = 0.f;
+#pragma unroll
+    for (int i = 0; i < 4; ++i) {
+        const int c = lane + i * 64;
+        if (c < n4) {
+            const float a = v[i].x - mean, bb = v[i].y - mean, cc = v[i].z - mean, dd = v[i].w - mean;
+            q += (a * a + bb * bb) + (cc * cc + dd * dd);
+        }
+    }
+    const float rstd = rsqrtf(wave_sum(q) / (float)D + eps);
+    const float one = add_one ? 1.0f : 0.0f;
+    To* yr = y + (size_t)row * ldy;
+#pragma unroll
+    for (int i = 0; i < 4; ++i) {
+        const int c = lane + i * 64;
+        if (c < n4) {
+            float4 ww = w ? *(const float4*)(w + c * 4) : make_float4(1.f - one, 1.f - one, 1.f - one, 1.f - one);
+            float4 bv = b ? *(const float4*)(b + c * 4) : make_float4(0.f, 0.f, 0.f, 0.f);
+            store4<To>(yr + c * 4, (v[i].x - mean) * rstd * (ww.x + one) + bv.x, (v[i].y - mean) * rstd * (ww.y + one) + bv.y,
+                       (v[i].z - mean) * rstd * (ww.z + one) + bv.z, (v[i].w - mean) * rstd * (ww.w + one) + bv.w);
+        }
+    }
+}
+
+template <typename To, typename Td>
+__device__ __forceinline__ void ln_row(const int row, const int lane, const LnRowArgs& a) {
+    ln_row<To, Td>(row, lane, a.x, a.ldx, (To*)a.y, a.ldy, a.R, a.D, a.w, a.b, a.add_one, a.eps, (const Td*)a.delta, a.ldd, (const Td*)a.delta2,
+                   a.keep_x, a.tail_row0, a.tp1, a.dt1, a.tp2, a.dt2);
+}
diff --git a/vietvoice-tts_amd/runtime.py b/vietvoice-tts_amd/runtime.py
--- a/vietvoice-tts_amd/runtime.py
+++ b/vietvoice-tts_amd/runtime.py
@@ -161,6 +161,7 @@
     "vv_gemm": (C.c_int, [C.c_void_p, C.POINTER(vv_gemm_args), C.c_void_p]),
     "vv_attention": (C.c_int, [C.c_void_p, C.POINTER(vv_attn_args), C.c_void_p]),
     "vv_layernorm": (C.c_int, [C.c_void_p, C.POINTER(vv_ln_args), C.c_void_p]),
+    "vv_attention_ln": (C.c_int, [C.c_void_p, C.POINTER(vv_attn_args), C.POINTER(vv_ln_args), C.c_void_p]),
     "vv_posconv": (C.c_int, [C.c_void_p, C.POINTER(vv_posconv_args), C.c_void_p]),
     "vv_conv1d": (C.c_int, [C.c_void_p, C.POINTER(vv_conv_args), C.c_void_p]),
     "vv_mrf_resblock": (C.c_int, [C.c_void_p, C.POINTER(vv_mrf_args), C.c_void_p]),
```

Result: slower. 183.8 (-5.6%).
